# ishine/minimax-speech

Measured on AMD Instinct MI355X. Metric: 24 kHz audio-seconds generated per wall-second per node (CosyVoice2-0.5B-shaped LM + flow + DAC-VAE, end to end), higher is better.
Workload: dtype bf16

## Files before the change

include/mmx_hip.h:

```cpp
#ifndef MMX_HIP_H
#define MMX_HIP_H
#include <stdint.h>
#ifdef __cplusplus
extern "C" {
#endif

#ifndef __HIP__
typedef struct ihipStream_t* hipStream_t;
#endif

#define MMX_F32 0
#define MMX_BF16 1
#define MMX_X2 2
#define MMX_X3 3
#define MMX_X2W 0x12
#define MMX_X3W 0x13
#define MMX_H2 4
#define MMX_H2W 0x14

#define MMX_ACT_NONE 0
#define MMX_ACT_LRELU 1
#define MMX_ACT_GELU 2
#define MMX_ACT_SILU 3
#define MMX_ACT_MISH 4
#define MMX_ACT_TANH 5

int mmx_abi_version(void);

typedef struct MmxGemmParams {
    const void* A;
    const void* W;
    const float* bias;
    const float* residual;
    const float* rowmask;
    const float* alpha;
    float* out_f32;
    void* out_act;
    int64_t lda, ldw, ldr, ldo_f, ldo_a;
    int64_t a_bstride, w_bstride, r_bstride, rm_bstride, of_bstride, oa_bstride;
    int64_t row_off, row_lo, row_hi;
    int64_t out_off, out_len;
    int32_t M, N, batch;
    int32_t ntaps, cin, dil;
    int32_t bias_mod, alpha_mod, bias_per_row;
    int32_t act, act2;
    float slope;
    int32_t row_stride;
} MmxGemmParams;
int mmx_gemm_win(const MmxGemmParams* p, int dtype, hipStream_t stream);
#define MMX_TILE_128x128 1
#define MMX_TILE_128x64 2
#define MMX_TILE_64x64 3
#define MMX_TILE_32x64 4
int mmx_gemm_win_tile(const MmxGemmParams* p, int dtype, int tile, hipStream_t stream);

int mmx_rownorm(const float* x, int64_t ldx, int64_t x_bstride, int rows, int C, int batch,
                const float* gamma, const float* beta, float eps, int rms, int act,
                const float* rowmask, int64_t rm_bstride, const float* addvec, int64_t av_bstride,
                float* out_f32, int64_t ldo_f, int64_t of_bstride,
                void* out_act, int64_t ldo_a, int64_t oa_bstride, int dtype, hipStream_t stream);

int mmx_groupnorm(const float* x, int B, int T, int C, int groups, const float* gamma, const float* beta, float eps,
                  int act, const float* rowmask, void* out, int dtype, hipStream_t stream);

int mmx_act_rows(const float* x, int64_t rows, int C, int act, const float* rowmask, float* out_f32, void* out_act, int dtype,
                 hipStream_t stream);

int mmx_gather_rows(const int64_t* ids, int n, const float* table, int C, float scale, const float* rowmask,
                    float* out_f32, int64_t ldo_f, void* out_act, int64_t ldo_a, int dtype, hipStream_t stream);

int mmx_copy2d(const void* in, int in_dtype, int64_t ibs, int64_t irs, int64_t ics, int rep,
               void* out, int out_dtype, int64_t obs, int64_t ors, int64_t ocs,
               int rows, int cols, int batch, hipStream_t stream);

int mmx_est_pack(const float* x, int64_t x_bs, int x_mod, const float* mu, const float* spks, const float* cond, int B, int T, int C,
                 void* h, int64_t ldh, int dtype, hipStream_t stream);
int mmx_sinusoidal_emb(const float* t, int B, int dim, float scale, void* out, int dtype, hipStream_t stream);

int mmx_cfg_euler(float* x, const float* d_cond, const float* d_uncond, float cfg, float dt, int64_t n,
                  hipStream_t stream);

int mmx_attn_dense(const void* q, int64_t ldq, int64_t q_bs, const void* k, int64_t ldk, int64_t k_bs,
                   const void* v, int64_t ldv, int64_t v_bs, void* out, int64_t ldo, int64_t o_bs,
                   int B, int H, int D, int Tq, int Tk, float scale, const float* keymask, int64_t km_bs, int chunk,
                   const void* pos, int64_t ldp, const float* pos_u, const float* pos_v,
                   int head_stride, int q_begin, int dtype, hipStream_t stream);
int mmx_attn_flash_bf16(const void* q, int64_t ldq, int64_t q_bs, const void* k, int64_t ldk, int64_t k_bs,
                        const void* vt, int64_t ldvt, int64_t vt_bs, void* out, int64_t ldo, int64_t o_bs,
                        int B, int H, int T, float scale, const float* keymask, int64_t km_bs, int chunk, int q_begin,
                        const int32_t* klen, hipStream_t stream);
int mmx_attn_relpos_x(const float* q, int64_t ldq, int64_t q_bs, const float* k, int64_t ldk, int64_t k_bs, const float* v,
                      int64_t ldv, int64_t v_bs, const float* pos, int64_t ldp, const float* pos_u, const float* pos_v,
                      float* out, int64_t ldo, int64_t o_bs, int B, int H, int T, float scale, int chunk, const int32_t* klen,
                      hipStream_t stream);
int mmx_attn_flash_x(const float* q, int64_t ldq, int64_t q_bs, const float* k, int64_t ldk, int64_t k_bs,
                     const float* v, int64_t ldv, int64_t v_bs, float* out, int64_t ldo, int64_t o_bs,
                     int B, int H, int T, float scale, const float* keymask, int64_t km_bs, int chunk,
                     int q_begin, const int32_t* klen, hipStream_t stream);
int mmx_attn_flash_xs(const void* qk, int64_t ldqk, int64_t qk_bs, const void* vt, int64_t ldvt, int64_t vt_bs,
                      float* out, int64_t ldo, int64_t o_bs, int B, int H, int T, float scale, const float* keymask,
                      int64_t km_bs, int chunk, int q_begin, const int32_t* klen, int form, hipStream_t stream);
int mmx_attn_relpos_bf16(const void* q, int64_t ldq, int64_t q_bs, const void* k, int64_t ldk, int64_t k_bs,
                         const void* vt, int64_t ldvt, int64_t vt_bs, const void* pos, int64_t ldp,
                         const float* pos_u, const float* pos_v, void* out, int64_t ldo, int64_t o_bs,
                         int B, int H, int T, float scale, int chunk, const int32_t* klen, hipStream_t stream);

int mmx_attn_flash_fp8(const void* q, int64_t ldq, int64_t q_bs, const void* k, int64_t ldk, int64_t k_bs,
                       const void* vt, int64_t ldvt, int64_t vt_bs, void* out, int64_t ldo, int64_t o_bs,
                       int B, int H, int T, float scale, const float* keymask, int64_t km_bs, int chunk, int q_begin,
                       const int32_t* klen, hipStream_t stream);

int mmx_conv_cin1(const float* x, int64_t x_bs, int T, int C, int k, const float* w, const float* bias, float slope,
                  const float* alpha, float* out_f32, void* out_act, int batch, int dtype, hipStream_t stream);
int mmx_vae_sample(const float* ml, const float* noise, int64_t rows, int D, float* z, float* m, float* logs,
                   hipStream_t stream);
int mmx_mask_rows(void* x, int64_t rows, int C, const float* rowmask, int dtype, hipStream_t stream);
int mmx_prefetch4(const void* p0, int64_t n0, const void* p1, int64_t n1, const void* p2, int64_t n2, const void* p3, int64_t n3,
                  void* sink, int workgroups, hipStream_t stream);
int mmx_resample_linear(const float* x, int64_t rows, int T, int T2, float* out, hipStream_t stream);

int mmx_conv_cout1_tanh(const void* act, int64_t a_bs, int T, int C, int k, const float* w, const float* bias,
                        float slope, int use_tanh, float* out, int64_t o_bs, int batch, int dtype, hipStream_t stream);

#define MMX_X_PACKED 1
#define MMX_OUT_PACKED 2
int mmx_pack_skinny(const void* w, int64_t ldw, int N, int K, const float* kscale, int interleave_half,
                    void* wp, int dtype, hipStream_t stream);
int mmx_skinny_gemm(const void* x, int x_dtype, int64_t ldx, int B, int K, int N, const void* wp,
                    const float* bias, int rs, float eps, int epi, float* out_f32, int64_t ldo_f,
                    void* out_act, int64_t ldo_a, int dtype, int flags, const float* kgamma, hipStream_t stream);

int mmx_decode_prep(const float* x, int64_t ldx, int B, int K, const float* gamma, float* h, int64_t ldh, void* xs,
                    float* ssq, int dtype, hipStream_t stream);
int mmx_skinny2(const void* xs, int B, int K, int N, const void* wp, const float* bias, const float* ssq_in, float eps,
                int epi, float* out, int64_t ldo, void* xs_out, const float* gamma_next, float* ssq_out,
                int tiles_per_wg, int ksplit, float* part, int64_t part_floats, int32_t* tickets, int dtype,
                hipStream_t stream);

int mmx_rope_kv_store(const float* qkv, int64_t ldqkv, int64_t qkv_bs, int B, int rows, int Hq, int Hkv, int D,
                      const float* inv_freq, const int32_t* pos, void* q_out, int64_t ldq, int64_t q_bs,
                      void* kc, void* vc, const int32_t* block_table, int max_pages, int page,
                      int dtype, hipStream_t stream);
int mmx_paged_attn(const void* q, int64_t ldq, int64_t q_bs, int B, int rows, int Hq, int Hkv, int D, float scale,
                   const int32_t* pos, const void* kc, const void* vc, const int32_t* block_table, int max_pages,
                   int page, void* out, int64_t ldo, int64_t o_bs, int dtype, hipStream_t stream);
int mmx_decode_attn(const float* qkv, int64_t ldqkv, int B, int Hq, int Hkv, int D, const float* inv_freq,
                    const float* rope_tab, const int32_t* pos, void* kc, void* vc, const int32_t* block_table, int max_pages, int page,
                    float scale, void* out, int64_t ldo, int dtype, int out_packed, hipStream_t stream);
int mmx_swiglu(const float* gu, int64_t ldgu, int rows, int I, void* out, int64_t ldo, int dtype, hipStream_t stream);

int mmx_sample_step(const float* logits, int64_t ldl, int V, int B, int eos_id, int top_k, float top_p,
                    int win_size, float tau_r, uint64_t seed, int32_t* state, int32_t* out_tokens, int max_out,
                    int32_t* sampled, const int32_t* forced, const float* speech_emb, int E, float* next_x,
                    int64_t ldx, float* logp_out, hipStream_t stream);

typedef struct MmxEstNext {
    const void* wqkv;
    const float* n1g;
    const float* n1b;
    void* q_out;
    void* vt_out;
    int64_t q_bs, vt_bs;
    int32_t ldq, ldvt;
} MmxEstNext;
typedef struct MmxEstTailParams {
    const void* ao;
    float* x;
    const void* wo;
    const void* w1;
    const void* w2;
    const float* bo;
    const float* b1;
    const float* b2;
    const float* n3g;
    const float* n3b;
    const float* rowmask;
    void* act_out;
    int64_t ao_bs, x_bs, rm_bs, act_bs;
    int32_t ldao, act_ld, B, T;
    int32_t t_begin;
    float eps;
    MmxEstNext next;
} MmxEstTailParams;
typedef struct MmxEstResnetParams {
    const void* a_in;
    float* x;
    const void* w1;
    const void* w2;
    const void* wr;
    const float* b1;
    const float* g1;
    const float* be1;
    const float* b2;
    const float* g2;
    const float* be2;
    const float* br;
    const float* tv;
    const float* rowmask;
    int64_t a_bs, x_bs, tv_bs, rm_bs;
    int32_t lda, cin, B, T;
    int32_t t_begin;
    float eps;
    MmxEstNext next;
} MmxEstResnetParams;
int mmx_est_tail(const MmxEstTailParams* p, int dtype, int bm, int cfg, hipStream_t stream);
int mmx_est_resnet(const MmxEstResnetParams* p, int dtype, int bm, int cfg, hipStream_t stream);
typedef struct {
    const float* x;
    float* x_out;
    void* act_out;
    const void* w7;
    const void* w1;
    const float* b7;
    const float* b1;
    const float* a0;
    const float* a2;
    const float* alpha_next;
    const int32_t* lens;
    int64_t x_bs;
    int32_t B, T, C, dil;
    float slope;
} MmxDacRuParams;
int mmx_dac_ru(const MmxDacRuParams* p, int dtype, int bm, hipStream_t stream);

#ifdef __cplusplus
}
#endif
#endif
```

minimax-speech_amd/csrc/common.h:

```cpp
#pragma once
#include <hip/hip_runtime.h>
#include <stdint.h>

#ifndef MMX_LAB
#define MMX_LAB 0
#endif
constexpr bool LAB = MMX_LAB != 0;

#define MMX_OK 0
#define MMX_EARG (-1)
#define MMX_CHECK_ARG(c) do { if (!(c)) return MMX_EARG; } while (0)
#define MMX_LAUNCH_CHECK() do { hipError_t e_ = hipGetLastError(); if (e_ != hipSuccess) return -(int)e_ - 1000; } while (0)

#define MMX_ACT_DTYPE(d) ((d) >= 2 ? 0 : (d))

#define MMX_LDS_OPT_IN(fn, bytes)                                                                                   \
    do {                                                                                                            \
        if ((bytes) > 64 * 1024) {                                                                                  \
            static bool done_[64] = {};                                                                             \
            int dev_ = 0;                                                                                           \
            if (hipGetDevice(&dev_) != hipSuccess || dev_ < 0 || dev_ >= 64) return MMX_EARG;                       \
            if (!done_[dev_]) {                                                                                     \
                hipError_t e_ = hipFuncSetAttribute((const void*)(fn), hipFuncAttributeMaxDynamicSharedMemorySize, 160 * 1024); \
                if (e_ != hipSuccess) return -1000 - (int)e_;                                                       \
                done_[dev_] = true;                                                                                 \
            }                                                                                                       \
        }                                                                                                           \
    } while (0)

typedef unsigned short bf16_t;
typedef __attribute__((ext_vector_type(8))) short short8_t;
typedef __attribute__((ext_vector_type(4))) float float4_t;
typedef __attribute__((ext_vector_type(4))) short short4_t;

__device__ __forceinline__ float bf2f(bf16_t v) { return __uint_as_float(((unsigned)v) << 16); }
__device__ __forceinline__ bf16_t f2bf(float f) { return __builtin_bit_cast(unsigned short, (__bf16)f); }
__device__ __forceinline__ unsigned pack_bf16x2(float lo, float hi) {
    typedef __attribute__((ext_vector_type(2))) __bf16 bf16x2_t;
    typedef __attribute__((ext_vector_type(2))) float f32x2_t;
    bf16x2_t v = __builtin_convertvector(f32x2_t{lo, hi}, bf16x2_t);
    return __builtin_bit_cast(unsigned, v);
}

template <typename T> struct Cvt;
template <> struct Cvt<float> {
    static __device__ __forceinline__ float to_f(float v) { return v; }
    static __device__ __forceinline__ float from_f(float v) { return v; }
};
template <> struct Cvt<bf16_t> {
    static __device__ __forceinline__ float to_f(bf16_t v) { return bf2f(v); }
    static __device__ __forceinline__ bf16_t from_f(float v) { return f2bf(v); }
};

template <int CTRL>
__device__ __forceinline__ float dpp_f32(float v) {
    return __builtin_bit_cast(float, __builtin_amdgcn_update_dpp(0, __builtin_bit_cast(int, v), CTRL, 0xf, 0xf, false));
}
__device__ __forceinline__ float group8_sum(float v) {
    v += dpp_f32<0xB1>(v);
    v += dpp_f32<0x4E>(v);
    v += dpp_f32<0x141>(v);
    return v;
}
__device__ __forceinline__ float group16_sum(float v) {
    v = group8_sum(v);
    v += dpp_f32<0x140>(v);
    return v;
}

__device__ __forceinline__ float wave_sum(float v) {
#pragma unroll
    for (int o = 32; o > 0; o >>= 1) v += __shfl_xor(v, o, 64);
    return v;
}
__device__ __forceinline__ float wave_max(float v) {
#pragma unroll
    for (int o = 32; o > 0; o >>= 1) v = fmaxf(v, __shfl_xor(v, o, 64));
    return v;
}

enum { ACT_NONE = 0, ACT_LRELU = 1, ACT_GELU = 2, ACT_SILU = 3, ACT_MISH = 4, ACT_TANH = 5 };

__device__ __forceinline__ float erf_fast(float x) {
    const float ax = fabsf(x);
    const float t = __builtin_amdgcn_rcpf(1.0f + 0.3275911f * ax);
    float p = 1.061405429f;
    p = p * t - 1.453152027f;
    p = p * t + 1.421413741f;
    p = p * t - 0.284496736f;
    p = p * t + 0.254829592f;
    const float r = 1.0f - p * t * __expf(-ax * ax);
    return copysignf(r, x);
}

typedef float f32x2_t __attribute__((ext_vector_type(2)));
__device__ __forceinline__ f32x2_t gelu_fast2(f32x2_t v) {
#pragma clang fp contract(off)
    const f32x2_t x = v * 0.70710678118654752f;
    const f32x2_t ax = __builtin_elementwise_abs(x);
    const f32x2_t d = __builtin_elementwise_fma(ax, (f32x2_t)(0.3275911f), (f32x2_t)(1.0f));
    f32x2_t t;
    t.x = __builtin_amdgcn_rcpf(d.x);
    t.y = __builtin_amdgcn_rcpf(d.y);
    f32x2_t p = (f32x2_t)(1.061405429f);
    p = __builtin_elementwise_fma(p, t, (f32x2_t)(-1.453152027f));
    p = __builtin_elementwise_fma(p, t, (f32x2_t)(1.421413741f));
    p = __builtin_elementwise_fma(p, t, (f32x2_t)(-0.284496736f));
    p = __builtin_elementwise_fma(p, t, (f32x2_t)(0.254829592f));
    const f32x2_t m = (ax * ax) * -1.4426950408889634f;
    f32x2_t e;
    e.x = __builtin_amdgcn_exp2f(m.x);
    e.y = __builtin_amdgcn_exp2f(m.y);
    const f32x2_t r = __builtin_elementwise_fma(-(p * t), e, (f32x2_t)(1.0f));
    f32x2_t er;
    er.x = __builtin_copysignf(r.x, x.x);
    er.y = __builtin_copysignf(r.y, x.y);
    return (v * 0.5f) * (er + 1.0f);
}

__device__ __forceinline__ float erf_poly(float x) {
    const float u = __builtin_fminf(__builtin_fmaxf(x, -3.0f), 3.0f);
    const float t = u * u;
    float p = 4.074212256e-08f;
    p = p * t - 1.944823225e-06f;
    p = p * t + 4.106053166e-05f;
    p = p * t - 5.110369530e-04f;
    p = p * t + 4.235427827e-03f;
    p = p * t - 2.510286123e-02f;
    p = p * t + 1.110793352e-01f;
    p = p * t - 3.753148615e-01f;
    p = p * t + 1.128268480e+00f;
    return u * p;
}

constexpr int ACT_GELU_POLY = 100;

template <int ACT, bool PRECISE>
__device__ __forceinline__ float act_c(float v, float slope) {
    if constexpr (ACT == ACT_LRELU) return v > 0.f ? v : v * slope;
    else if constexpr (ACT == ACT_GELU_POLY) return 0.5f * v * (1.f + erf_poly(v * 0.70710678118654752f));
    else if constexpr (ACT == ACT_GELU) return 0.5f * v * (1.f + (PRECISE ? erff(v * 0.70710678118654752f) : erf_fast(v * 0.70710678118654752f)));
    else if constexpr (ACT == ACT_SILU) return v / (1.f + (PRECISE ? expf(-v) : __expf(-v)));
    else if constexpr (ACT == ACT_MISH) {
        if (v > 20.f) return v;
        const float e = PRECISE ? expf(v) : __expf(v);
        const float n = e * (e + 2.f);
        return v * (n / (n + 2.f));
    } else if constexpr (ACT == ACT_TANH) return tanhf(v);
    else return v;
}

template <bool PRECISE>
__device__ __forceinline__ float act_apply(float v, int act, float slope) {
    switch (act) {
        case ACT_LRELU: return v > 0.f ? v : v * slope;
        case ACT_GELU: return 0.5f * v * (1.f + erff(v * 0.70710678118654752f));
        case ACT_SILU: return v / (1.f + (PRECISE ? expf(-v) : __expf(-v)));
        case ACT_MISH: {
            float sp = v > 20.f ? v : log1pf(PRECISE ? expf(v) : __expf(v));
            return v * tanhf(sp);
        }
        case ACT_TANH: return tanhf(v);
        default: return v;
    }
}

__device__ __forceinline__ float sin_cw(float x) {
    const float n = __builtin_rintf(x * 0.318309886183790672f);
    float r = __builtin_fmaf(-n, 3.14159274101257324f, x);
    r = __builtin_fmaf(-n, -8.74227765734758577e-8f, r);
    const float t = r * r;
    float p = -2.3846693509e-08f;
    p = p * t + 2.7522619348e-06f;
    p = p * t - 1.9840804453e-04f;
    p = p * t + 8.3333300427e-03f;
    p = p * t - 1.6666667163e-01f;
    const float s = __builtin_fmaf(r * t, p, r);
    return (static_cast<int>(n) & 1) ? -s : s;
}

template <bool PRECISE>
__device__ __forceinline__ float snake_apply(float x, float alpha) {
    float s = PRECISE ? sin_cw(alpha * x) : __sinf(alpha * x);
    return x + (1.0f / (alpha + 1e-9f)) * (s * s);
}
```

minimax-speech_amd/csrc/decode.hip:

```cpp
#include "common.h"
#include "../../include/mmx_hip.h"

namespace {

typedef __attribute__((ext_vector_type(4))) unsigned int u32x4_t;
typedef __attribute__((ext_vector_type(8))) _Float16 half8_t;
constexpr float H2_WSCALE = 256.f;

__device__ __forceinline__ void st_sc1(float* p, float v) { __hip_atomic_store(p, v, __ATOMIC_RELAXED, __HIP_MEMORY_SCOPE_AGENT); }
__device__ __forceinline__ float ld_sc1(const float* p) { return __hip_atomic_load(p, __ATOMIC_RELAXED, __HIP_MEMORY_SCOPE_AGENT); }

constexpr unsigned OOB = 0x80000000u;
constexpr int SSQ_SLOTS = 64;

__device__ __forceinline__ int plane_index(int row, int col, int nkb) {
    return (((((row >> 4) * nkb + (col >> 5)) << 6) + (((col & 31) >> 3) << 4) + (row & 15)) << 3) + (col & 7);
}
template <int NS, bool F16 = false>
__device__ __forceinline__ void store_split(bf16_t* planes, int ps, int idx, float v) {
#pragma unroll
    for (int s = 0; s < NS; ++s) {
        if constexpr (F16) {
            const _Float16 h = (_Float16)v;
            planes[s * ps + idx] = __builtin_bit_cast(unsigned short, h);
            v -= (float)h;
        } else {
            const bf16_t h = f2bf(v);
            planes[s * ps + idx] = h;
            v -= bf2f(h);
        }
    }
}
template <bool F16>
__device__ __forceinline__ float4_t mma16(u32x4_t a, u32x4_t b, float4_t c) {
    if constexpr (F16) return __builtin_amdgcn_mfma_f32_16x16x32_f16(__builtin_bit_cast(half8_t, a), __builtin_bit_cast(half8_t, b), c, 0, 0, 0);
    else return __builtin_amdgcn_mfma_f32_16x16x32_bf16(__builtin_bit_cast(short8_t, a), __builtin_bit_cast(short8_t, b), c, 0, 0, 0);
}

struct Skinny3Args {
    const bf16_t* xs;
    const bf16_t* wp;
    const float* bias;
    const float* ssq_in;
    float* out;
    bf16_t* xs_out;
    const float* gamma_next;
    float* ssq_out;
    float* part;
    int* tickets;
    long ldo;
    int B, K, N, ntiles, kb_per_wg;
    float eps;
    unsigned wplane;
    float wscale;
};

__device__ unsigned long long* g_skinny_stamps = nullptr;
#define STAMP(i) do { if constexpr (LAB) { if (stamps && lane == 0) stamps[((blockIdx.y * gridDim.x + blockIdx.x) * 8 + wave) * 8 + (i)] = __builtin_amdgcn_s_memtime(); } } while (0)

template <int MT, int TW, int KPW, int EPI, int NS, int NWP = 1, bool F16 = false>
__global__ __launch_bounds__(512) void skinny3_kernel(Skinny3Args a) {
    unsigned long long* stamps = nullptr;
    unsigned long long t_entry = 0;
    if constexpr (LAB) { t_entry = __builtin_amdgcn_s_memtime(); stamps = g_skinny_stamps; }
    constexpr int NB = EPI == 1 ? 2 : 1;
    constexpr int PER = TW * NB * MT * 4;
    extern __shared__ __attribute__((aligned(16))) char smem[];
    float* red = reinterpret_cast<float*>(smem);
    float* rstd = red + 8 * PER * 64;
    const int lane = threadIdx.x & 63;
    const int wave = __builtin_amdgcn_readfirstlane(threadIdx.x >> 6);
    const int g = lane >> 4, l16 = lane & 15;
    const int J = gridDim.y, j = blockIdx.y;
    const int nkb = a.K >> 5;
    const int wkb0 = j * a.kb_per_wg, wkb1 = min(nkb, wkb0 + a.kb_per_wg);
    const int wn = wkb1 - wkb0;
    const int kb0 = wkb0 + ((wn * wave) >> 3), kb1 = wkb0 + ((wn * (wave + 1)) >> 3);
    const int tile0 = blockIdx.x * TW;
    const int ntiles = a.ntiles;

    STAMP(0);
    if constexpr (LAB) { if (stamps && lane == 0) stamps[((blockIdx.y * gridDim.x + blockIdx.x) * 8 + wave) * 8 + 7] = t_entry; }
    const auto w_rsrc = __builtin_amdgcn_make_buffer_rsrc(const_cast<bf16_t*>(a.wp), 0, 0x7fffffff, 0x00020000);
    const auto x_rsrc = __builtin_amdgcn_make_buffer_rsrc(const_cast<bf16_t*>(a.xs), 0, 0x7fffffff, 0x00020000);
    const unsigned voff = lane * 16;
    u32x4_t wf[NWP][TW][NB][KPW];
#pragma unroll
    for (int p2 = 0; p2 < NWP; ++p2)
#pragma unroll
        for (int t = 0; t < TW; ++t)
#pragma unroll
            for (int n = 0; n < NB; ++n)
#pragma unroll
                for (int i = 0; i < KPW; ++i) {
                    const bool ok = tile0 + t < ntiles && kb0 + i < kb1;
                    const unsigned so = ok ? ((unsigned)(((tile0 + t) * NB + n) * nkb + kb0 + i) << 10) + p2 * a.wplane : OOB;
                    wf[p2][t][n][i] = __builtin_amdgcn_raw_buffer_load_b128(w_rsrc, voff, so, 2);
                }
    u32x4_t xf[NS][KPW][MT];
#pragma unroll
    for (int s = 0; s < NS; ++s)
#pragma unroll
        for (int i = 0; i < KPW; ++i)
#pragma unroll
            for (int m = 0; m < MT; ++m) {
                const unsigned so = kb0 + i < kb1 ? ((unsigned)((s * MT + m) * nkb + kb0 + i) << 10) : OOB;
                xf[s][i][m] = __builtin_amdgcn_raw_buffer_load_b128(x_rsrc, voff, so, 0);
            }
    if (a.ssq_in) {
        const int row = threadIdx.x >> 4, part = threadIdx.x & 15;
        const float4 q = *reinterpret_cast<const float4*>(a.ssq_in + row * SSQ_SLOTS + part * 4);
        float sq = group16_sum((q.x + q.y) + (q.z + q.w));
        if (part == 0) rstd[row] = rsqrtf(sq / (float)a.K + a.eps);
    }
    constexpr int UNITS = TW * MT * 4, UPW = (UNITS + 7) / 8;
    float pre_bias[UPW], pre_gn[UPW], pre_res[UPW];
#pragma unroll
    for (int k = 0; k < UPW; ++k) {
        const int u = wave + 8 * k, t = u / (MT * 4), m = (u / 4) % MT, r = u & 3;
        const int row = m * 16 + 4 * g + r, ncol = (tile0 + t) * 16 + l16;
        const bool ok = u < UNITS && tile0 + t < ntiles && row < a.B && ncol < a.N;
        pre_bias[k] = (EPI != 1 && a.bias && ok) ? a.bias[ncol] : 0.f;
        pre_gn[k] = (EPI == 2 && a.gamma_next && ok) ? a.gamma_next[ncol] : 1.f;
        pre_res[k] = (EPI == 2 && ok) ? a.out[(long)row * a.ldo + ncol] : 0.f;
    }
    STAMP(1);
    if constexpr (LAB) { if (stamps) { asm volatile("s_waitcnt vmcnt(0)" ::: "memory"); STAMP(2); } }
    float4_t acc[TW][NB][MT];
#pragma unroll
    for (int t = 0; t < TW; ++t)
#pragma unroll
        for (int n = 0; n < NB; ++n)
#pragma unroll
            for (int m = 0; m < MT; ++m) acc[t][n][m] = float4_t{0.f, 0.f, 0.f, 0.f};
#pragma unroll
    for (int i = 0; i < KPW; ++i)
#pragma unroll
        for (int t = 0; t < TW; ++t)
#pragma unroll
            for (int n = 0; n < NB; ++n)
#pragma unroll
                for (int p2 = 0; p2 < NWP; ++p2) {
#pragma unroll
                    for (int m = 0; m < MT; ++m)
#pragma unroll
                        for (int s = 0; s < NS; ++s) {
                            if (s + p2 >= NS) continue;
                            acc[t][n][m] = mma16<F16>(xf[s][i][m], wf[p2][t][n][i], acc[t][n][m]);
                        }
                }
    {
        float* mine = red + wave * PER * 64 + lane;
#pragma unroll
        for (int t = 0; t < TW; ++t)
#pragma unroll
            for (int n = 0; n < NB; ++n)
#pragma unroll
                for (int m = 0; m < MT; ++m)
#pragma unroll
                    for (int r = 0; r < 4; ++r) mine[(((t * NB + n) * MT + m) * 4 + r) * 64] = acc[t][n][m][r];
    }
    STAMP(3);
    __syncthreads();
    STAMP(4);
    float sum[UPW][NB];
#pragma unroll
    for (int k = 0; k < UPW; ++k) {
        const int u = wave + 8 * k, t = u / (MT * 4), m = (u / 4) % MT, r = u & 3;
#pragma unroll
        for (int n = 0; n < NB; ++n) {
            float v = 0.f;
            if (u < UNITS) {
#pragma unroll
                for (int w2 = 0; w2 < 8; ++w2) v += red[w2 * PER * 64 + (((t * NB + n) * MT + m) * 4 + r) * 64 + lane];
            }
            sum[k][n] = v;
        }
    }
    if constexpr (EPI == 2) {
        if (J > 1) {
            int* flag = reinterpret_cast<int*>(rstd + 32);
#pragma unroll
            for (int k = 0; k < UPW; ++k) {
                const int u = wave + 8 * k;
                if (u < UNITS) st_sc1(a.part + ((j * gridDim.x + blockIdx.x) * UNITS + u) * 64 + lane, sum[k][0]);
            }
            asm volatile("s_waitcnt vmcnt(0)" ::: "memory");
            __syncthreads();
            if (threadIdx.x == 0) {
                const int old = __hip_atomic_fetch_add(a.tickets + blockIdx.x, 1, __ATOMIC_RELAXED, __HIP_MEMORY_SCOPE_AGENT);
                if (old == J - 1) __hip_atomic_store(a.tickets + blockIdx.x, 0, __ATOMIC_RELAXED, __HIP_MEMORY_SCOPE_AGENT);
                *flag = old == J - 1;
            }
            __syncthreads();
            STAMP(5);
            if (!*flag) return;
            constexpr int JMAX = 8;
            float pv[UPW][JMAX];
#pragma unroll
            for (int k = 0; k < UPW; ++k)
#pragma unroll
                for (int j2 = 0; j2 < JMAX; ++j2) {
                    const int u = min(wave + 8 * k, UNITS - 1), jc = min(j2, J - 1);
                    const float v = ld_sc1(a.part + ((jc * gridDim.x + blockIdx.x) * UNITS + u) * 64 + lane);
                    pv[k][j2] = j2 < J ? v : 0.f;
                }
#pragma unroll
            for (int k = 0; k < UPW; ++k) {
                float v = 0.f;
#pragma unroll
                for (int j2 = 0; j2 < JMAX; ++j2) v += pv[k][j2];
                sum[k][0] = v;
            }
        }
    }
    const int nkb_out = a.N >> 5;
    const int ps_out = MT * nkb_out * 512;
#pragma unroll
    for (int k = 0; k < UPW; ++k) {
        const int u = wave + 8 * k, t = u / (MT * 4), m = (u / 4) % MT, r = u & 3;
        if (u >= UNITS) break;
        const int row = m * 16 + 4 * g + r, tile = tile0 + t, ncol = tile * 16 + l16;
        const float sc = (a.ssq_in ? rstd[row] : 1.f) * a.wscale;
        const bool ok = tile < ntiles && row < a.B && ncol < a.N;
        if constexpr (EPI == 1) {
            const float gte = sum[k][0] * sc, up = sum[k][1] * sc;
            if (ok) store_split<NS, F16>(a.xs_out, ps_out, plane_index(row, ncol, nkb_out), gte / (1.f + expf(-gte)) * up);
        } else {
            float vv = sum[k][0] * sc + pre_bias[k];
            if constexpr (EPI == 2) vv += pre_res[k];
            if (ok) a.out[(long)row * a.ldo + ncol] = vv;
            if constexpr (EPI == 2) {
                if (ok && a.xs_out) store_split<NS, F16>(a.xs_out, ps_out, plane_index(row, ncol, nkb_out), vv * pre_gn[k]);
                if (a.ssq_out) {
                    const float q = group16_sum(ok ? vv * vv : 0.f);
                    if (l16 == 0 && tile < ntiles) a.ssq_out[row * SSQ_SLOTS + tile] = q;
                }
            }
        }
    }
    STAMP(6);
}

template <int MT, int TW, int KPW, int EPI, int NS, int NWP = 1, bool F16 = false>
int launch(const Skinny3Args& a, int J, hipStream_t s) {
    constexpr int NB = EPI == 1 ? 2 : 1;
    const size_t lds = (size_t)8 * (TW * NB * MT * 4) * 64 * sizeof(float) + 32 * sizeof(float) + 16;
    MMX_LDS_OPT_IN((skinny3_kernel<MT, TW, KPW, EPI, NS, NWP, F16>), lds);
    dim3 grid((a.ntiles + TW - 1) / TW, J);
    hipLaunchKernelGGL((skinny3_kernel<MT, TW, KPW, EPI, NS, NWP, F16>), grid, dim3(512), lds, s, a);
    MMX_LAUNCH_CHECK();
    return MMX_OK;
}

template <int NS, bool F16 = false>
__global__ __launch_bounds__(256) void decode_prep_kernel(const float* __restrict__ x, long ldx, int B, int K, const float* __restrict__ gamma,
                                                          float* __restrict__ h, long ldh, bf16_t* __restrict__ xs, int mt,
                                                          float* __restrict__ ssq) {
    const int row = blockIdx.x, nkb = K >> 5;
    const int ps = mt * nkb * 512;
    for (int t0 = threadIdx.x; t0 < SSQ_SLOTS * 16; t0 += 256) {
        const int tile = t0 >> 4, col = t0;
        float v = 0.f;
        if (col < K) {
            v = x[(long)row * ldx + col];
            if (h) h[(long)row * ldh + col] = v;
            store_split<NS, F16>(xs, ps, plane_index(row, col, nkb), v * (gamma ? gamma[col] : 1.f));
        }
        const float q = group16_sum(v * v);
        if ((t0 & 15) == 0) ssq[row * SSQ_SLOTS + tile] = q;
    }
}

}

extern "C" int mmx_decode_prep(const float* x, int64_t ldx, int B, int K, const float* gamma, float* h, int64_t ldh, void* xs,
                               float* ssq, int dtype, hipStream_t stream) {
    MMX_CHECK_ARG(x && xs && ssq && B > 0 && B <= 32 && K > 0 && K % 32 == 0 && K <= SSQ_SLOTS * 16 && (dtype == MMX_X3 || dtype == MMX_BF16 || dtype == MMX_H2));
    if (dtype == MMX_H2) hipLaunchKernelGGL((decode_prep_kernel<2, true>), dim3(B), dim3(256), 0, stream, x, ldx, B, K, gamma, h, ldh, (bf16_t*)xs, (B + 15) / 16, ssq);
    else if (dtype == MMX_X3) hipLaunchKernelGGL(decode_prep_kernel<3>, dim3(B), dim3(256), 0, stream, x, ldx, B, K, gamma, h, ldh, (bf16_t*)xs, (B + 15) / 16, ssq);
    else hipLaunchKernelGGL(decode_prep_kernel<1>, dim3(B), dim3(256), 0, stream, x, ldx, B, K, gamma, h, ldh, (bf16_t*)xs, (B + 15) / 16, ssq);
    MMX_LAUNCH_CHECK();
    return MMX_OK;
}

extern "C" int mmx_skinny2(const void* xs, int B, int K, int N, const void* wp, const float* bias, const float* ssq_in, float eps,
                           int epi, float* out, int64_t ldo, void* xs_out, const float* gamma_next, float* ssq_out,
                           int tiles_per_wg, int ksplit, float* part, int64_t part_floats, int32_t* tickets, int dtype,
                           hipStream_t stream) {
    MMX_CHECK_ARG(xs && wp && B > 0 && B <= 32 && K > 0 && K % 32 == 0 && N > 0 &&
                  (dtype == MMX_X3 || dtype == MMX_X3W || dtype == MMX_BF16 || dtype == MMX_H2 || dtype == MMX_H2W));
    MMX_CHECK_ARG(dtype != MMX_X3W || tiles_per_wg == 1);
    MMX_CHECK_ARG(((uintptr_t)xs % 16) == 0 && ((uintptr_t)wp % 16) == 0 && (!ssq_in || ((uintptr_t)ssq_in % 16) == 0));
    MMX_CHECK_ARG(ksplit >= 1 && ksplit <= 8 && (ksplit == 1 || (epi == 2 && part && tickets)));
    MMX_CHECK_ARG(epi == 1 ? (xs_out != nullptr && N % 32 == 0) : out != nullptr);
    MMX_CHECK_ARG(epi != 2 || !xs_out || N % 32 == 0);
    MMX_CHECK_ARG(epi != 2 || !ssq_out || (N + 15) / 16 <= SSQ_SLOTS);
    const int nkb = K / 32, ntiles = (N + 15) / 16, mt = (B + 15) / 16;
    const int per_wave = ((nkb + ksplit - 1) / ksplit + 7) / 8;
    MMX_CHECK_ARG(ksplit == 1 || part_floats >= (int64_t)ksplit * ((ntiles + tiles_per_wg - 1) / tiles_per_wg) * tiles_per_wg * mt * 4 * 64);
    const double plane_bytes = (double)ntiles * (epi == 1 ? 2 : 1) * nkb * 1024.0;
    MMX_CHECK_ARG(plane_bytes * (dtype == MMX_X3W ? 3 : (dtype == MMX_H2W ? 2 : 1)) < 2147483000.0);
    const bool f16 = dtype == MMX_H2 || dtype == MMX_H2W;
    Skinny3Args a{(const bf16_t*)xs, (const bf16_t*)wp, bias, ssq_in, out, (bf16_t*)xs_out, gamma_next, ssq_out, part, tickets,
                  ldo, B, K, N, ntiles, (nkb + ksplit - 1) / ksplit, eps, (unsigned)plane_bytes, f16 ? 1.0f / H2_WSCALE : 1.0f};
#define GO(MT, TW, KPW, EPI) do { if (dtype == MMX_X3) return launch<MT, TW, KPW, EPI, 3>(a, ksplit, stream); \
                                  if (dtype == MMX_H2) return launch<MT, TW, KPW, EPI, 2, 1, true>(a, ksplit, stream); \
                                  if (dtype == MMX_H2W) return launch<MT, TW, KPW, EPI, 2, 2, true>(a, ksplit, stream); \
                                  if (dtype == MMX_X3W) { if constexpr (TW == 1) return launch<MT, 1, KPW, EPI, 3, 3>(a, ksplit, stream); else return MMX_EARG; } \
                                  return launch<MT, TW, KPW, EPI, 1>(a, ksplit, stream); } while (0)
#define BY_MT(TW, KPW, EPI) do { if (mt == 1) GO(1, TW, KPW, EPI); else GO(2, TW, KPW, EPI); } while (0)
    if (per_wave <= 4) {
        if (epi == 0) { if (tiles_per_wg == 1) BY_MT(1, 4, 0); if (tiles_per_wg == 2) BY_MT(2, 4, 0); }
        if (epi == 1) { if (tiles_per_wg == 1) BY_MT(1, 4, 1); if (tiles_per_wg == 2) BY_MT(2, 4, 1); }
        if (epi == 2) { if (tiles_per_wg == 1) BY_MT(1, 4, 2); if (tiles_per_wg == 2) BY_MT(2, 4, 2); }
    }
#undef BY_MT
#undef GO
    return MMX_EARG;
}

#if MMX_LAB
extern "C" int mmx_lab_skinny_stamps(void* buf) {
    unsigned long long* p = reinterpret_cast<unsigned long long*>(buf);
    const hipError_t e = hipMemcpyToSymbol(HIP_SYMBOL(g_skinny_stamps), &p, sizeof(p));
    return e == hipSuccess ? MMX_OK : -(int)e - 1000;
}
#endif
```

minimax-speech_amd/csrc/llm.hip:

```cpp
#include "common.h"
#include "../../include/mmx_hip.h"

template <typename T>
__global__ void pack_skinny_kernel(const T* __restrict__ w, long ldw, int N, int K, const float* __restrict__ kscale,
                                   int half, T* __restrict__ wp) {
    constexpr int E = sizeof(T) == 2 ? 8 : 4;
    constexpr int KB = E * 4;
    const long total = (long)((N + 15) / 16) * (K / KB) * 64 * E;
    for (long idx = (long)blockIdx.x * blockDim.x + threadIdx.x; idx < total; idx += (long)gridDim.x * blockDim.x) {
        int j = idx % E;
        long t = idx / E;
        int lane = t % 64;
        t /= 64;
        int kb = t % (K / KB);
        int tile = t / (K / KB);
        int col = lane & 15, g = lane >> 4;
        int row;
        if (half > 0) row = (tile & 1) * half + (tile >> 1) * 16 + col;
        else row = tile * 16 + col;
        int kk = kb * KB + g * E + j;
        float v = 0.f;
        if (row < N && (half == 0 || ((tile >> 1) * 16 + col) < half)) {
            v = Cvt<T>::to_f(w[(long)row * ldw + kk]);
            if (kscale) v *= kscale[kk];
        }
        wp[idx] = Cvt<T>::from_f(v);
    }
}
extern "C" int mmx_pack_skinny(const void* w, int64_t ldw, int N, int K, const float* kscale, int interleave_half,
                               void* wp, int dtype, hipStream_t stream) {
    MMX_CHECK_ARG(w && wp && N > 0 && K > 0 && K % 32 == 0);
    MMX_CHECK_ARG(interleave_half == 0 || (N == 2 * interleave_half && interleave_half % 16 == 0));
    if (dtype == MMX_X2 || dtype == MMX_X3) { MMX_CHECK_ARG(!kscale); dtype = MMX_BF16; }
    if (dtype == MMX_BF16) hipLaunchKernelGGL(pack_skinny_kernel<bf16_t>, dim3(2048), dim3(256), 0, stream, (const bf16_t*)w, ldw, N, K, kscale, interleave_half, (bf16_t*)wp);
    else if (dtype == MMX_F32) hipLaunchKernelGGL(pack_skinny_kernel<float>, dim3(2048), dim3(256), 0, stream, (const float*)w, ldw, N, K, kscale, interleave_half, (float*)wp);
    else return MMX_EARG;
    MMX_LAUNCH_CHECK();
    return MMX_OK;
}

template <typename T>
__device__ __forceinline__ long act_packed_index(int row, int col, int K) {
    constexpr int E = sizeof(T) == 2 ? 8 : 4, KB = 4 * E;
    const int kb = col / KB, g = (col % KB) / E, j = col % E;
    return ((((long)(row >> 4) * (K / KB) + kb) * 64) + g * 16 + (row & 15)) * E + j;
}

template <typename T, typename TX, int MT, int EPI, int KS, bool XPK, bool OPK, int NS = 1>
__global__ __launch_bounds__(512) void skinny_gemm_kernel(const TX* __restrict__ x, long ldx, int B, int K, int N,
                                   const T* __restrict__ wp, const float* __restrict__ bias, int rs, float eps,
                                   float* __restrict__ outf, long ldo_f, T* __restrict__ outa, long ldo_a,
                                   int ksplit, int ntiles, const float* __restrict__ kgamma) {
    constexpr bool BF = sizeof(T) == 2;
    static_assert(NS == 1 || (BF && sizeof(TX) == 4 && !XPK && !OPK), "split build: bf16 weights, fp32 row-major activations");
    constexpr int E = BF ? 8 : 4;
    constexpr int KB = E * 4;
    constexpr int NB = EPI == 1 ? 2 : 1;
    constexpr int XV = sizeof(TX) == 4 ? E / 4 : 1;
    typedef __attribute__((ext_vector_type(4))) unsigned int u32x4_t;
    extern __shared__ __attribute__((aligned(16))) char smem[];
    float* red = reinterpret_cast<float*>(smem);
    const int lane = threadIdx.x & 63, wave = threadIdx.x >> 6;
    const int nwaves = blockDim.x >> 6;
    const int g = lane >> 4, l16 = lane & 15;
    const int tpb = nwaves / ksplit;
    const int tile = blockIdx.x * tpb + wave / ksplit;
    const int ksl = wave % ksplit;
    const int nkb = K / KB;
    const int kb_per = (nkb + ksplit - 1) / ksplit;
    const int kb0 = ksl * kb_per, kb1 = min(nkb, kb0 + kb_per);
    const bool active = tile < ntiles;

    float4_t acc[NB][MT];
#pragma unroll
    for (int n = 0; n < NB; ++n)
#pragma unroll
        for (int m = 0; m < MT; ++m) acc[n][m] = float4_t{0.f, 0.f, 0.f, 0.f};
    float ssq[MT];
#pragma unroll
    for (int m = 0; m < MT; ++m) ssq[m] = 0.f;
    constexpr bool SSQ_MFMA = BF && sizeof(TX) == 2 && EPI != 2;
    float4_t accd[MT];
#pragma unroll
    for (int m = 0; m < MT; ++m) accd[m] = float4_t{0.f, 0.f, 0.f, 0.f};
    float pre_bias = 0.f, pre_res[MT][4];
    if (active && ksl == 0) {
        const int n = tile * 16 + l16;
        if (EPI != 1 && bias && n < N) pre_bias = bias[n];
        if constexpr (EPI == 2) {
#pragma unroll
            for (int m = 0; m < MT; ++m)
#pragma unroll
                for (int r = 0; r < 4; ++r) {
                    const int row = m * 16 + 4 * g + r;
                    pre_res[m][r] = (row < B && n < N) ? outf[(long)row * ldo_f + n] : 0.f;
                }
        }
    }

    if (active) {
        const T* wbase = wp + ((long)tile * NB * nkb) * 64 * E + (long)lane * E;
        for (int kc = kb0; kc < kb1; kc += KS) {
            u32x4_t wf[KS][NB];
#pragma unroll
            for (int i = 0; i < KS; ++i)
#pragma unroll
                for (int n = 0; n < NB; ++n)
                    if (kc + i < kb1)
                        wf[i][n] = __builtin_nontemporal_load(reinterpret_cast<const u32x4_t*>(wbase + ((long)n * nkb + kc + i) * 64 * E));
            u32x4_t xr[KS][MT][XV];
#pragma unroll
            for (int i = 0; i < KS; ++i)
#pragma unroll
                for (int m = 0; m < MT; ++m)
#pragma unroll
                    for (int v = 0; v < XV; ++v) {
                        if constexpr (XPK)
                            xr[i][m][v] = (kc + i < kb1)
                                              ? *reinterpret_cast<const u32x4_t*>(x + (((long)m * nkb + kc + i) * 64 + lane) * E)
                                              : u32x4_t{0, 0, 0, 0};
                        else
                            xr[i][m][v] = (kc + i < kb1 && m * 16 + l16 < B)
                                              ? *reinterpret_cast<const u32x4_t*>(reinterpret_cast<const char*>(x + (long)(m * 16 + l16) * ldx + (kc + i) * KB + g * E) + v * 16)
                                              : u32x4_t{0, 0, 0, 0};
                    }
#pragma unroll
            for (int i = 0; i < KS; ++i) {
                if (kc + i >= kb1) continue;
#pragma unroll
                for (int m = 0; m < MT; ++m) {
                    float xv[E];
                    u32x4_t raw[XV];
#pragma unroll
                    for (int v = 0; v < XV; ++v) raw[v] = xr[i][m][v];
                    if constexpr (sizeof(TX) == 4) {
#pragma unroll
                        for (int e = 0; e < E; ++e) xv[e] = __uint_as_float(raw[e / 4][e % 4]);
                    } else {
#pragma unroll
                        for (int e = 0; e < E; ++e) xv[e] = __uint_as_float((raw[0][e / 2] >> ((e & 1) * 16)) << 16);
                    }
                    if constexpr (SSQ_MFMA) {
                        if (rs) {
                            const short8_t xf = *reinterpret_cast<const short8_t*>(&raw[0]);
                            accd[m] = __builtin_amdgcn_mfma_f32_16x16x32_bf16(xf, xf, accd[m], 0, 0, 0);
                        }
                    } else if (rs) {
#pragma unroll
                        for (int e = 0; e < E; ++e) ssq[m] += xv[e] * xv[e];
                    }
                    if constexpr (NS > 1 || (BF && sizeof(TX) == 4)) {
                        if (kgamma) {
                            const float4 g0 = *reinterpret_cast<const float4*>(kgamma + (kc + i) * KB + g * E);
                            const float4 g1 = *reinterpret_cast<const float4*>(kgamma + (kc + i) * KB + g * E + 4);
                            xv[0] *= g0.x; xv[1] *= g0.y; xv[2] *= g0.z; xv[3] *= g0.w;
                            xv[4] *= g1.x; xv[5] *= g1.y; xv[6] *= g1.z; xv[7] *= g1.w;
                        }
#pragma unroll
                        for (int s2 = 0; s2 < NS; ++s2) {
                            short8_t af;
#pragma unroll
                            for (int e = 0; e < 8; ++e) {
                                const bf16_t hb = f2bf(xv[e]);
                                af[e] = (short)hb;
                                xv[e] -= bf2f(hb);
                            }
#pragma unroll
                            for (int n = 0; n < NB; ++n) {
                                short8_t bfr = *reinterpret_cast<const short8_t*>(&wf[i][n]);
                                acc[n][m] = __builtin_amdgcn_mfma_f32_16x16x32_bf16(af, bfr, acc[n][m], 0, 0, 0);
                            }
                        }
                    } else if constexpr (BF) {
                        short8_t af;
                        if constexpr (sizeof(TX) == 2) {
                            af = *reinterpret_cast<const short8_t*>(&raw[0]);
                        } else {
#pragma unroll
                            for (int e = 0; e < 8; ++e) af[e] = (short)f2bf(xv[e]);
                        }
#pragma unroll
                        for (int n = 0; n < NB; ++n) {
                            short8_t bfr = *reinterpret_cast<const short8_t*>(&wf[i][n]);
                            acc[n][m] = __builtin_amdgcn_mfma_f32_16x16x32_bf16(af, bfr, acc[n][m], 0, 0, 0);
                        }
                    } else {
#pragma unroll
                        for (int n = 0; n < NB; ++n) {
                            float4_t bfr = *reinterpret_cast<const float4_t*>(&wf[i][n]);
#pragma unroll
                            for (int s2 = 0; s2 < 4; ++s2)
                                acc[n][m] = __builtin_amdgcn_mfma_f32_16x16x4f32(xv[s2], bfr[s2], acc[n][m], 0, 0, 0);
                        }
                    }
                }
            }
        }
    }
    if constexpr (SSQ_MFMA) {
        if (rs) {
#pragma unroll
            for (int m = 0; m < MT; ++m) {
                const int r = l16 & 3;
                const float d = r == 0 ? accd[m][0] : (r == 1 ? accd[m][1] : (r == 2 ? accd[m][2] : accd[m][3]));
                ssq[m] = (l16 >> 2) == g ? d : 0.f;
            }
        }
    }
    if (rs) {
#pragma unroll
        for (int m = 0; m < MT; ++m) {
            ssq[m] += __shfl_xor(ssq[m], 16, 64);
            ssq[m] += __shfl_xor(ssq[m], 32, 64);
        }
    }
    constexpr int PER = NB * MT * 4 + MT;
    if (ksplit > 1) {
        float* mine = red + ((long)wave * PER) * 64 + lane;
#pragma unroll
        for (int n = 0; n < NB; ++n)
#pragma unroll
            for (int m = 0; m < MT; ++m)
#pragma unroll
                for (int r = 0; r < 4; ++r) mine[((n * MT + m) * 4 + r) * 64] = acc[n][m][r];
#pragma unroll
        for (int m = 0; m < MT; ++m) mine[(NB * MT * 4 + m) * 64] = ssq[m];
        __syncthreads();
        if (ksl != 0) return;
        for (int w2 = 1; w2 < ksplit; ++w2) {
            const float* o = red + ((long)(wave + w2) * PER) * 64 + lane;
#pragma unroll
            for (int n = 0; n < NB; ++n)
#pragma unroll
                for (int m = 0; m < MT; ++m)
#pragma unroll
                    for (int r = 0; r < 4; ++r) acc[n][m][r] += o[((n * MT + m) * 4 + r) * 64];
#pragma unroll
            for (int m = 0; m < MT; ++m) ssq[m] += o[(NB * MT * 4 + m) * 64];
        }
    }
    if (!active) return;
#pragma unroll
    for (int m = 0; m < MT; ++m) {
#pragma unroll
        for (int r = 0; r < 4; ++r) {
            const int row = m * 16 + 4 * g + r;
            float sc = 1.f;
            if (rs) {
                float sq = __shfl(ssq[m], 4 * g + r, 64);
                sc = rsqrtf(sq / (float)K + eps);
            }
            if (row >= B) continue;
            if constexpr (EPI == 1) {
                const int n = tile * 16 + l16;
                if (n < N) {
                    float gte = acc[0][m][r] * sc, up = acc[1][m][r] * sc;
                    float sl = gte / (1.f + expf(-gte));
                    if constexpr (NS > 1) outf[(long)row * ldo_f + n] = sl * up;
                    else outa[OPK ? act_packed_index<T>(row, n, N) : (long)row * ldo_a + n] = Cvt<T>::from_f(sl * up);
                }
            } else {
                const int n = tile * 16 + l16;
                if (n < N) {
                    float v = acc[0][m][r] * sc + pre_bias;
                    if constexpr (EPI == 2) v += pre_res[m][r];
                    if (outf) outf[(long)row * ldo_f + n] = v;
                    if constexpr (NS == 1)
                        if (outa) outa[OPK ? act_packed_index<T>(row, n, N) : (long)row * ldo_a + n] = Cvt<T>::from_f(v);
                }
            }
        }
    }
}

template <typename T, typename TX, int EPI, bool XPK, bool OPK, int NS = 1>
static int skinny_launch_mt(const void* x, int64_t ldx, int B, int K, int N, const void* wp, const float* bias, int rs,
                            float eps, float* outf, int64_t ldo_f, void* outa, int64_t ldo_a, hipStream_t s,
                            const float* kgamma = nullptr) {
    constexpr int KB = sizeof(T) == 2 ? 32 : 16;
    const int ntiles = (N + 15) / 16;
    const int nkb = K / KB;
    const int mt = (B + 15) / 16;
    const int KSr = mt == 1 ? 10 : (mt == 2 ? 7 : 4);
    int ksplit = 1;
    while (ksplit < 8 && (nkb + ksplit - 1) / ksplit > KSr) ksplit *= 2;
    int waves = ksplit >= 4 ? ksplit : 4;
    if (mt >= 2 && ksplit <= 4 && ntiles >= 256) waves = 8;
    int tpb = waves / ksplit;
    dim3 grid((ntiles + tpb - 1) / tpb), block(waves * 64);
    constexpr int NB = EPI == 1 ? 2 : 1;
    size_t lds = ksplit > 1 ? (size_t)waves * (NB * mt * 4 + mt) * 64 * 4 : 0;
#define SK(MT) hipLaunchKernelGGL((skinny_gemm_kernel<T, TX, MT, EPI, (MT == 1 ? 10 : (MT == 2 ? 7 : 4)), XPK, OPK, NS>), grid, block, lds, s, (const TX*)x, ldx, B, K, N, (const T*)wp, \
        bias, rs, eps, outf, ldo_f, (T*)outa, ldo_a, ksplit, ntiles, kgamma)
    switch (mt) {
        case 1: SK(1); break;
        case 2: SK(2); break;
        case 3: SK(3); break;
        case 4: SK(4); break;
        default: return MMX_EARG;
    }
#undef SK
    MMX_LAUNCH_CHECK();
    return MMX_OK;
}
template <typename T, typename TX, bool XPK, bool OPK>
static int skinny_launch_epi(int epi, const void* x, int64_t ldx, int B, int K, int N, const void* wp, const float* bias,
                             int rs, float eps, float* outf, int64_t ldo_f, void* outa, int64_t ldo_a, hipStream_t s) {
    if (epi == 0) return skinny_launch_mt<T, TX, 0, XPK, OPK>(x, ldx, B, K, N, wp, bias, rs, eps, outf, ldo_f, outa, ldo_a, s);
    if (epi == 1) return skinny_launch_mt<T, TX, 1, XPK, OPK>(x, ldx, B, K, N, wp, bias, rs, eps, outf, ldo_f, outa, ldo_a, s);
    if (epi == 2) return skinny_launch_mt<T, TX, 2, XPK, OPK>(x, ldx, B, K, N, wp, bias, rs, eps, outf, ldo_f, outa, ldo_a, s);
    return MMX_EARG;
}
template <typename T, typename TX>
static int skinny_launch_layout(int flags, int epi, const void* x, int64_t ldx, int B, int K, int N, const void* wp,
                                const float* bias, int rs, float eps, float* outf, int64_t ldo_f, void* outa, int64_t ldo_a,
                                hipStream_t s) {
    if constexpr (sizeof(T) == sizeof(TX)) {
        if (flags == (MMX_X_PACKED | MMX_OUT_PACKED))
            return skinny_launch_epi<T, TX, true, true>(epi, x, ldx, B, K, N, wp, bias, rs, eps, outf, ldo_f, outa, ldo_a, s);
        if (flags == MMX_X_PACKED)
            return skinny_launch_epi<T, TX, true, false>(epi, x, ldx, B, K, N, wp, bias, rs, eps, outf, ldo_f, outa, ldo_a, s);
    }
    if (flags == 0) return skinny_launch_epi<T, TX, false, false>(epi, x, ldx, B, K, N, wp, bias, rs, eps, outf, ldo_f, outa, ldo_a, s);
    return MMX_EARG;
}
template <int NS>
static int skinny_launch_split(int epi, const void* x, int64_t ldx, int B, int K, int N, const void* wp, const float* bias, int rs,
                               float eps, float* outf, int64_t ldo_f, hipStream_t s, const float* kgamma) {
    if (epi == 0) return skinny_launch_mt<bf16_t, float, 0, false, false, NS>(x, ldx, B, K, N, wp, bias, rs, eps, outf, ldo_f, nullptr, 0, s, kgamma);
    if (epi == 1) return skinny_launch_mt<bf16_t, float, 1, false, false, NS>(x, ldx, B, K, N, wp, bias, rs, eps, outf, ldo_f, nullptr, 0, s, kgamma);
    if (epi == 2) return skinny_launch_mt<bf16_t, float, 2, false, false, NS>(x, ldx, B, K, N, wp, bias, rs, eps, outf, ldo_f, nullptr, 0, s, kgamma);
    return MMX_EARG;
}
extern "C" int mmx_skinny_gemm(const void* x, int x_dtype, int64_t ldx, int B, int K, int N, const void* wp,
                               const float* bias, int rs, float eps, int epi, float* out_f32, int64_t ldo_f,
                               void* out_act, int64_t ldo_a, int dtype, int flags, const float* kgamma, hipStream_t stream) {
    MMX_CHECK_ARG(x && wp && B > 0 && B <= 64 && K > 0 && K % 32 == 0 && N > 0);
    if (dtype == MMX_X2 || dtype == MMX_X3) {
        MMX_CHECK_ARG(x_dtype == MMX_F32 && flags == 0 && out_f32 && !out_act && ldx % 8 == 0 && ((uintptr_t)x % 16) == 0 && ((uintptr_t)wp % 16) == 0);
        MMX_CHECK_ARG(!kgamma || ((uintptr_t)kgamma % 16) == 0);
        return dtype == MMX_X2 ? skinny_launch_split<2>(epi, x, ldx, B, K, N, wp, bias, rs, eps, out_f32, ldo_f, stream, kgamma)
                               : skinny_launch_split<3>(epi, x, ldx, B, K, N, wp, bias, rs, eps, out_f32, ldo_f, stream, kgamma);
    }
    if (kgamma) {
        MMX_CHECK_ARG(dtype == MMX_BF16 && x_dtype == MMX_F32 && flags == 0 && ((uintptr_t)kgamma % 16) == 0 && ldx % 8 == 0 && ((uintptr_t)x % 16) == 0);
        if (epi == 0) return skinny_launch_mt<bf16_t, float, 0, false, false, 1>(x, ldx, B, K, N, wp, bias, rs, eps, out_f32, ldo_f, out_act, ldo_a, stream, kgamma);
        if (epi == 1) return skinny_launch_mt<bf16_t, float, 1, false, false, 1>(x, ldx, B, K, N, wp, bias, rs, eps, out_f32, ldo_f, out_act, ldo_a, stream, kgamma);
        return MMX_EARG;
    }
    MMX_CHECK_ARG((flags == 0 || flags == MMX_X_PACKED || flags == (MMX_X_PACKED | MMX_OUT_PACKED)) && (flags == 0 || x_dtype == dtype) &&
                  (!(flags & MMX_OUT_PACKED) || N % 32 == 0));
    MMX_CHECK_ARG(ldx % 8 == 0 && ((uintptr_t)x % 16) == 0 && ((uintptr_t)wp % 16) == 0);
    MMX_CHECK_ARG(epi == 1 ? out_act != nullptr : (out_f32 != nullptr || (epi == 0 && out_act != nullptr)));
    MMX_CHECK_ARG(epi != 2 || out_f32 != nullptr);
    if (dtype == MMX_BF16) {
        if (x_dtype == MMX_F32) return skinny_launch_layout<bf16_t, float>(flags, epi, x, ldx, B, K, N, wp, bias, rs, eps, out_f32, ldo_f, out_act, ldo_a, stream);
        if (x_dtype == MMX_BF16) return skinny_launch_layout<bf16_t, bf16_t>(flags, epi, x, ldx, B, K, N, wp, bias, rs, eps, out_f32, ldo_f, out_act, ldo_a, stream);
    } else if (dtype == MMX_F32 && x_dtype == MMX_F32) {
        return skinny_launch_layout<float, float>(flags, epi, x, ldx, B, K, N, wp, bias, rs, eps, out_f32, ldo_f, out_act, ldo_a, stream);
    }
    return MMX_EARG;
}

template <typename T>
__global__ void rope_kv_kernel(const float* __restrict__ qkv, long ldqkv, long qkv_bs, int Hq, int Hkv,
                               const float* __restrict__ inv_freq, const int32_t* __restrict__ pos,
                               T* __restrict__ q_out, long ldq, long q_bs, T* __restrict__ kc, T* __restrict__ vc,
                               const int32_t* __restrict__ block_table, int max_pages, int page) {
    constexpr int D = 64, HALF = 32;
    const int b = blockIdx.y, t = blockIdx.x;
    const int p = pos[b] + t;
    const float* src = qkv + (long)b * qkv_bs + (long)t * ldqkv;
    const int nh = Hq + 2 * Hkv;
    const int phys = block_table[(long)b * max_pages + p / page];
    const int slot = p % page;
    for (int i = threadIdx.x; i < nh * HALF; i += blockDim.x) {
        const int hh = i / HALF, d = i % HALF;
        const float x0 = src[hh * D + d], x1 = src[hh * D + d + HALF];
        float y0 = x0, y1 = x1;
        if (hh < Hq + Hkv) {
            const float ang = (float)p * inv_freq[d];
            const float c = cosf(ang), s = sinf(ang);
            y0 = x0 * c - x1 * s;
            y1 = x1 * c + x0 * s;
        }
        if (hh < Hq) {
            T* o = q_out + (long)b * q_bs + (long)t * ldq + hh * D;
            o[d] = Cvt<T>::from_f(y0);
            o[d + HALF] = Cvt<T>::from_f(y1);
        } else {
            const int hk = (hh - Hq) % Hkv;
            T* base = (hh < Hq + Hkv ? kc : vc) + (((long)phys * Hkv + hk) * page + slot) * D;
            base[d] = Cvt<T>::from_f(y0);
            base[d + HALF] = Cvt<T>::from_f(y1);
        }
    }
}
extern "C" int mmx_rope_kv_store(const float* qkv, int64_t ldqkv, int64_t qkv_bs, int B, int rows, int Hq, int Hkv, int D,
                                 const float* inv_freq, const int32_t* pos, void* q_out, int64_t ldq, int64_t q_bs,
                                 void* kc, void* vc, const int32_t* block_table, int max_pages, int page,
                                 int dtype, hipStream_t stream) {
    dtype = MMX_ACT_DTYPE(dtype);
    MMX_CHECK_ARG(qkv && inv_freq && pos && q_out && kc && vc && block_table && B > 0 && rows > 0 && D == 64 && page > 0);
    dim3 grid(rows, B);
    if (dtype == MMX_BF16) hipLaunchKernelGGL(rope_kv_kernel<bf16_t>, grid, dim3(256), 0, stream, qkv, ldqkv, qkv_bs, Hq, Hkv, inv_freq, pos, (bf16_t*)q_out, ldq, q_bs, (bf16_t*)kc, (bf16_t*)vc, block_table, max_pages, page);
    else if (dtype == MMX_F32) hipLaunchKernelGGL(rope_kv_kernel<float>, grid, dim3(256), 0, stream, qkv, ldqkv, qkv_bs, Hq, Hkv, inv_freq, pos, (float*)q_out, ldq, q_bs, (float*)kc, (float*)vc, block_table, max_pages, page);
    else return MMX_EARG;
    MMX_LAUNCH_CHECK();
    return MMX_OK;
}

template <typename T>
__global__ __launch_bounds__(256) void paged_attn_kernel(
    const T* __restrict__ q, long ldq, long q_bs, int Hq, int Hkv, float scale, const int32_t* __restrict__ pos,
    const T* __restrict__ kc, const T* __restrict__ vc, const int32_t* __restrict__ block_table, int max_pages,
    int page, T* __restrict__ out, long ldo, long o_bs) {
    constexpr int D = 64;
    extern __shared__ __attribute__((aligned(16))) char smem[];
    float* qs = reinterpret_cast<float*>(smem);
    float* red = qs + D;
    float* S = red + 8 + 4 * D;
    const int tid = threadIdx.x, lane = tid & 63, wave = tid >> 6;
    const int h = blockIdx.x, t = blockIdx.y, b = blockIdx.z;
    const int hk = h / (Hq / Hkv);
    const int ctx = pos[b] + t + 1;
    const int32_t* bt = block_table + (long)b * max_pages;
    if (tid < D) qs[tid] = Cvt<T>::to_f(q[(long)b * q_bs + (long)t * ldq + h * D + tid]);
    __syncthreads();
    float mx = -INFINITY;
    for (int j = tid; j < ctx; j += 256) {
        const T* kp = kc + (((long)bt[j / page] * Hkv + hk) * page + j % page) * D;
        float s = 0.f;
#pragma unroll
        for (int d = 0; d < D; ++d) s += qs[d] * Cvt<T>::to_f(kp[d]);
        s *= scale;
        S[j] = s;
        mx = fmaxf(mx, s);
    }
    mx = wave_max(mx);
    if (lane == 0) red[wave] = mx;
    __syncthreads();
    mx = fmaxf(fmaxf(red[0], red[1]), fmaxf(red[2], red[3]));
    float l = 0.f;
    for (int j = tid; j < ctx; j += 256) {
        float e = expf(S[j] - mx);
        S[j] = e;
        l += e;
    }
    l = wave_sum(l);
    if (lane == 0) red[4 + wave] = l;
    __syncthreads();
    l = red[4] + red[5] + red[6] + red[7];
    float acc = 0.f;
    for (int j = wave; j < ctx; j += 4) {
        const T* vp = vc + (((long)bt[j / page] * Hkv + hk) * page + j % page) * D;
        acc += S[j] * Cvt<T>::to_f(vp[lane]);
    }
    red[8 + wave * D + lane] = acc;
    __syncthreads();
    if (wave == 0) {
        float o = (red[8 + lane] + red[8 + D + lane]) + (red[8 + 2 * D + lane] + red[8 + 3 * D + lane]);
        out[(long)b * o_bs + (long)t * ldo + h * D + lane] = Cvt<T>::from_f(o / l);
    }
}
extern "C" int mmx_paged_attn(const void* q, int64_t ldq, int64_t q_bs, int B, int rows, int Hq, int Hkv, int D, float scale,
                              const int32_t* pos, const void* kc, const void* vc, const int32_t* block_table, int max_pages,
                              int page, void* out, int64_t ldo, int64_t o_bs, int dtype, hipStream_t stream) {
    dtype = MMX_ACT_DTYPE(dtype);
    MMX_CHECK_ARG(q && pos && kc && vc && block_table && out && B > 0 && rows > 0 && D == 64 && Hq % Hkv == 0 && page > 0);
    const size_t max_ctx = (size_t)max_pages * page;
    size_t lds = (64 + 8 + 4 * 64 + max_ctx) * 4;
    MMX_CHECK_ARG(lds <= 160 * 1024);
    dim3 grid(Hq, rows, B);
    if (dtype == MMX_BF16) hipLaunchKernelGGL(paged_attn_kernel<bf16_t>, grid, dim3(256), lds, stream, (const bf16_t*)q, ldq, q_bs, Hq, Hkv, scale, pos, (const bf16_t*)kc, (const bf16_t*)vc, block_table, max_pages, page, (bf16_t*)out, ldo, o_bs);
    else if (dtype == MMX_F32) hipLaunchKernelGGL(paged_attn_kernel<float>, grid, dim3(256), lds, stream, (const float*)q, ldq, q_bs, Hq, Hkv, scale, pos, (const float*)kc, (const float*)vc, block_table, max_pages, page, (float*)out, ldo, o_bs);
    else return MMX_EARG;
    MMX_LAUNCH_CHECK();
    return MMX_OK;
}

template <typename T>
__device__ __forceinline__ void load8(const T* p, float o[8]) {
    if constexpr (sizeof(T) == 2) {
        uint4 r = *reinterpret_cast<const uint4*>(p);
        const unsigned w[4] = {r.x, r.y, r.z, r.w};
#pragma unroll
        for (int i = 0; i < 4; ++i) {
            o[2 * i] = __uint_as_float(w[i] << 16);
            o[2 * i + 1] = __uint_as_float(w[i] & 0xffff0000u);
        }
    } else {
        float4 a = *reinterpret_cast<const float4*>(p), b = *reinterpret_cast<const float4*>(p + 4);
        o[0] = a.x; o[1] = a.y; o[2] = a.z; o[3] = a.w; o[4] = b.x; o[5] = b.y; o[6] = b.z; o[7] = b.w;
    }
}
template <typename T>
struct Raw8 {
    uint4 a, b;
    __device__ __forceinline__ void load(const T* p) {
        a = *reinterpret_cast<const uint4*>(p);
        if constexpr (sizeof(T) == 4) b = *reinterpret_cast<const uint4*>(p + 4);
    }
    __device__ __forceinline__ void to_float(float o[8]) const {
        const unsigned w[4] = {a.x, a.y, a.z, a.w};
        if constexpr (sizeof(T) == 2) {
#pragma unroll
            for (int i = 0; i < 4; ++i) {
                o[2 * i] = __uint_as_float(w[i] << 16);
                o[2 * i + 1] = __uint_as_float(w[i] & 0xffff0000u);
            }
        } else {
            const unsigned w2[4] = {b.x, b.y, b.z, b.w};
#pragma unroll
            for (int i = 0; i < 4; ++i) { o[i] = __uint_as_float(w[i]); o[4 + i] = __uint_as_float(w2[i]); }
        }
    }
};

template <typename T, int OM, int HP>
__global__ __launch_bounds__(256) void decode_attn_kernel(
    const float* __restrict__ qkv, long ldqkv, int Hq, int Hkv, const float* __restrict__ inv_freq,
    const float* __restrict__ rope_tab, const int32_t* __restrict__ pos, T* __restrict__ kc, T* __restrict__ vc,
    const int32_t* __restrict__ block_table, int max_pages, int page, float scale, T* __restrict__ out, long ldo,
    int nseq) {
    constexpr int D = 64, HALF = 32, NG = 32;
    extern __shared__ __attribute__((aligned(16))) char smem[];
    float* qs = reinterpret_cast<float*>(smem);
    float* kn = qs + HP * D;
    float* vn = kn + D;
    float* gm = vn + D;
    float* gl = gm + HP * NG;
    float* part = gl + HP * NG;
    int* bts = reinterpret_cast<int*>(part + HP * NG * D);
    const int tid = threadIdx.x;
    const int group = Hq / Hkv, nsub = (group + HP - 1) / HP;
    const int xcd = blockIdx.x & 7, slot = blockIdx.x >> 3;
    const int kvg = (slot / nsub) * 8 + xcd;
    if (kvg >= Hkv * nseq) return;
    const int b = kvg / Hkv, hk = kvg % Hkv, sub = slot % nsub;
    const int h0 = hk * group + sub * HP, nh = min(HP, group - sub * HP);
    const int32_t* bt = block_table + (long)b * max_pages;
    for (int i = tid; i < max_pages; i += 256) bts[i] = bt[i];
    const int p = pos[b];
    const float* src = qkv + (long)b * ldqkv;
    const float sc2 = scale * 1.44269504088896341f;
    if (tid < (HP + 1) * HALF) {
        const int which = tid >> 5, d = tid & 31;
        const float* x = src + (which < HP ? (h0 + min(which, nh - 1)) * D : (Hq + hk) * D);
        float c, s;
        if (rope_tab) {
            c = rope_tab[(long)p * D + d];
            s = rope_tab[(long)p * D + HALF + d];
        } else {
            const float ang = (float)p * inv_freq[d];
            c = cosf(ang);
            s = sinf(ang);
        }
        const float y0 = x[d] * c - x[d + HALF] * s, y1 = x[d + HALF] * c + x[d] * s;
        if (which < HP) { qs[which * D + d] = y0 * sc2; qs[which * D + d + HALF] = y1 * sc2; }
        else { kn[d] = Cvt<T>::to_f(Cvt<T>::from_f(y0)); kn[d + HALF] = Cvt<T>::to_f(Cvt<T>::from_f(y1)); }
    } else if (tid < (HP + 1) * HALF + D) {
        const int d = tid - (HP + 1) * HALF;
        vn[d] = Cvt<T>::to_f(Cvt<T>::from_f(src[(Hq + Hkv + hk) * D + d]));
    }
    __syncthreads();
    if (sub == 0 && tid < D) {
        const long o = (((long)bts[p / page] * Hkv + hk) * page + p % page) * D + tid;
        kc[o] = Cvt<T>::from_f(kn[tid]);
        vc[o] = Cvt<T>::from_f(vn[tid]);
    }
    const int kg = tid >> 3, dc = tid & 7;
    float qv[HP][8];
#pragma unroll
    for (int hp = 0; hp < HP; ++hp)
#pragma unroll
        for (int e = 0; e < 8; ++e) qv[hp][e] = qs[hp * D + dc * 8 + e];
    float m[HP], l[HP], acc[HP][8];
#pragma unroll
    for (int hp = 0; hp < HP; ++hp) {
        m[hp] = -INFINITY;
        l[hp] = 0.f;
#pragma unroll
        for (int e = 0; e < 8; ++e) acc[hp][e] = 0.f;
    }
    auto consume = [&](const float kv[8], const float vv[8]) {
#pragma unroll
        for (int hp = 0; hp < HP; ++hp) {
            float sdot = 0.f;
#pragma unroll
            for (int e = 0; e < 8; ++e) sdot = __builtin_fmaf(qv[hp][e], kv[e], sdot);
            sdot = group8_sum(sdot);
            const float mn = fmaxf(m[hp], sdot);
            const float al = __builtin_amdgcn_exp2f(m[hp] - mn), pj = __builtin_amdgcn_exp2f(sdot - mn);
            l[hp] = __builtin_fmaf(l[hp], al, pj);
#pragma unroll
            for (int e = 0; e < 8; ++e) acc[hp][e] = __builtin_fmaf(acc[hp][e], al, pj * vv[e]);
            m[hp] = mn;
        }
    };
    constexpr int U = sizeof(T) == 2 ? 12 : 10;
    for (int j0 = kg; j0 < p; j0 += NG * U) {
        Raw8<T> rk[U], rv[U];
#pragma unroll
        for (int u = 0; u < U; ++u) {
            const int j = j0 + u * NG;
            if (j < p) {
                const long o = (((long)bts[j / page] * Hkv + hk) * page + j % page) * D + dc * 8;
                rk[u].load(kc + o);
                rv[u].load(vc + o);
            }
        }
#pragma unroll
        for (int u = 0; u < U; ++u) {
            if (j0 + u * NG < p) {
                float kv[8], vv[8];
                rk[u].to_float(kv);
                rv[u].to_float(vv);
                consume(kv, vv);
            }
        }
    }
    if (kg == p % NG) {
        float kv[8], vv[8];
#pragma unroll
        for (int e = 0; e < 8; ++e) { kv[e] = kn[dc * 8 + e]; vv[e] = vn[dc * 8 + e]; }
        consume(kv, vv);
    }
#pragma unroll
    for (int hp = 0; hp < HP; ++hp) {
        if (dc == 0) { gm[hp * NG + kg] = m[hp]; gl[hp * NG + kg] = l[hp]; }
#pragma unroll
        for (int e = 0; e < 8; ++e) part[(hp * NG + kg) * D + dc * 8 + e] = acc[hp][e];
    }
    __syncthreads();
    if (tid < nh * D) {
        const int hp = tid >> 6, d = tid & 63, h = h0 + hp;
        const float* gmh = gm + hp * NG;
        const float* glh = gl + hp * NG;
        const float* ph = part + hp * NG * D;
        float M = -INFINITY;
#pragma unroll
        for (int g2 = 0; g2 < NG; ++g2) M = fmaxf(M, gmh[g2]);
        float L = 0.f, o = 0.f;
#pragma unroll
        for (int g2 = 0; g2 < NG; ++g2) {
            const float w = __builtin_amdgcn_exp2f(gmh[g2] - M);
            L = __builtin_fmaf(glh[g2], w, L);
            o = __builtin_fmaf(ph[g2 * D + d], w, o);
        }
        if constexpr (OM == 2) {
            const int nkb = Hq * D / 32, col = h * D + d;
            const long ps = (long)((nseq + 15) / 16) * nkb * 512;
            const long idx = ((((long)(b >> 4) * nkb + (col >> 5)) * 64) + (((col & 31) >> 3) << 4) + (b & 15)) * 8 + (col & 7);
            bf16_t* pl = reinterpret_cast<bf16_t*>(out);
            const float v = o / L;
            const bf16_t hh = f2bf(v);
            const float r1 = v - bf2f(hh);
            const bf16_t mm = f2bf(r1);
            pl[idx] = hh;
            pl[ps + idx] = mm;
            pl[2 * ps + idx] = f2bf(r1 - bf2f(mm));
        } else if constexpr (OM == 3) {
            const int nkb = Hq * D / 32, col = h * D + d;
            const long ps = (long)((nseq + 15) / 16) * nkb * 512;
            const long idx = ((((long)(b >> 4) * nkb + (col >> 5)) * 64) + (((col & 31) >> 3) << 4) + (b & 15)) * 8 + (col & 7);
            unsigned short* pl = reinterpret_cast<unsigned short*>(out);
            const float v = o / L;
            const _Float16 hh = (_Float16)v;
            pl[idx] = __builtin_bit_cast(unsigned short, hh);
            pl[ps + idx] = __builtin_bit_cast(unsigned short, (_Float16)(v - (float)hh));
        } else {
            out[OM == 1 ? act_packed_index<T>(b, h * D + d, Hq * D) : (long)b * ldo + h * D + d] = Cvt<T>::from_f(o / L);
        }
    }
}

template <bool OPK, int G>
__global__ __launch_bounds__(256) void decode_attn_gqa_kernel(
    const float* __restrict__ qkv, long ldqkv, int Hq, int Hkv, const float* __restrict__ inv_freq,
    const float* __restrict__ rope_tab, const int32_t* __restrict__ pos, bf16_t* __restrict__ kc, bf16_t* __restrict__ vc,
    const int32_t* __restrict__ block_table, int max_pages, float scale, bf16_t* __restrict__ out, long ldo, int nseq) {
    constexpr int D = 64, HALF = 32, PAGE = 16, NS = 8;
    static_assert(G <= 8, "one 8-float row of P per key");
    extern __shared__ __attribute__((aligned(16))) char smem[];
    bf16_t* qh = reinterpret_cast<bf16_t*>(smem);
    bf16_t* ql = qh + 16 * D;
    bf16_t* kn = ql + 16 * D;
    bf16_t* vn = kn + D;
    float* Pw = reinterpret_cast<float*>(vn + D);
    float* Aw = Pw + 4 * NS * 16 * 8;
    float* gm = Aw + 32;
    float* gl = gm + 32;
    float* part = gl + 32;
    int* bts = reinterpret_cast<int*>(part + 32 * G * D);
    const int tid = threadIdx.x, wave = tid >> 6, lane = tid & 63, l16 = lane & 15, g = lane >> 4;
    const int b = blockIdx.x / Hkv, hk = blockIdx.x % Hkv;
    const int32_t* bt = block_table + (long)b * max_pages;
    const int p = pos[b];
    const int NT = p / PAGE + 1;
    for (int i = tid; i < NT; i += 256) bts[i] = bt[i];
    for (int i = tid; i < 2 * 16 * D / 2; i += 256) reinterpret_cast<unsigned*>(qh)[i] = 0u;
    __syncthreads();
    const float* src = qkv + (long)b * ldqkv;
    const float sc2 = scale * 1.44269504088896341f;
    {
        const int which = tid >> 5, d = tid & 31;
        if (which <= G) {
            const float* x = src + (which < G ? (hk * G + which) * D : (Hq + hk) * D);
            float c, s;
            if (rope_tab) {
                c = rope_tab[(long)p * D + d];
                s = rope_tab[(long)p * D + HALF + d];
            } else {
                const float ang = (float)p * inv_freq[d];
                c = cosf(ang);
                s = sinf(ang);
            }
            const float y0 = x[d] * c - x[d + HALF] * s, y1 = x[d + HALF] * c + x[d] * s;
            if (which < G) {
                const float a0 = y0 * sc2, a1 = y1 * sc2;
                const bf16_t h0 = f2bf(a0), h1 = f2bf(a1);
                qh[which * D + d] = h0;
                qh[which * D + d + HALF] = h1;
                ql[which * D + d] = f2bf(a0 - bf2f(h0));
                ql[which * D + d + HALF] = f2bf(a1 - bf2f(h1));
            } else {
                kn[d] = f2bf(y0);
                kn[d + HALF] = f2bf(y1);
            }
        }
        if (tid < D) vn[tid] = f2bf(src[(Hq + Hkv + hk) * D + tid]);
    }
    __syncthreads();
    if (tid < D) {
        const long o = (((long)bts[p / PAGE] * Hkv + hk) * PAGE + p % PAGE) * D + tid;
        kc[o] = kn[tid];
        vc[o] = vn[tid];
    }
    short8_t bqh[2], bql[2];
#pragma unroll
    for (int ks = 0; ks < 2; ++ks) {
        bqh[ks] = *reinterpret_cast<const short8_t*>(qh + l16 * D + ks * 32 + 8 * g);
        bql[ks] = *reinterpret_cast<const short8_t*>(ql + l16 * D + ks * 32 + 8 * g);
    }
    const int ksub = lane >> 3, dc = lane & 7;
    const int tp = p / PAGE, rp = p % PAGE;
    float* Pme = Pw + wave * NS * 16 * 8;
    float m_run = -INFINITY, l_part = 0.f;
    typedef __attribute__((ext_vector_type(2))) float float2_t;
    float2_t acc[G][4];
#pragma unroll
    for (int h = 0; h < G; ++h)
#pragma unroll
        for (int e = 0; e < 4; ++e) acc[h][e] = float2_t{0.f, 0.f};

    for (int r0 = 0; r0 < NT; r0 += 4 * NS) {
        if (r0 + wave >= NT) break;
        uint4 rk[NS][2], rv[NS][2];
#pragma unroll
        for (int i = 0; i < NS; ++i) {
            const int t = r0 + 4 * i + wave;
            if (t < NT) {
                const long base = ((long)bts[t] * Hkv + hk) * PAGE * D;
#pragma unroll
                for (int ks = 0; ks < 2; ++ks) rk[i][ks] = *reinterpret_cast<const uint4*>(kc + base + l16 * D + ks * 32 + 8 * g);
#pragma unroll
                for (int hf = 0; hf < 2; ++hf) rv[i][hf] = *reinterpret_cast<const uint4*>(vc + base + (ksub + 8 * hf) * D + dc * 8);
            }
        }
        float4_t sacc[NS];
        float bm = -INFINITY;
#pragma unroll
        for (int i = 0; i < NS; ++i) {
            const int t = r0 + 4 * i + wave;
            sacc[i] = float4_t{-INFINITY, -INFINITY, -INFINITY, -INFINITY};
            if (t < NT) {
                if (t == tp) {
                    if (l16 == rp) {
#pragma unroll
                        for (int ks = 0; ks < 2; ++ks) rk[i][ks] = *reinterpret_cast<const uint4*>(kn + ks * 32 + 8 * g);
                    }
#pragma unroll
                    for (int hf = 0; hf < 2; ++hf) {
                        if (ksub + 8 * hf == rp) rv[i][hf] = *reinterpret_cast<const uint4*>(vn + dc * 8);
                        if (ksub + 8 * hf > rp) rv[i][hf] = make_uint4(0u, 0u, 0u, 0u);
                    }
                }
                float4_t c = {0.f, 0.f, 0.f, 0.f};
#pragma unroll
                for (int ks = 0; ks < 2; ++ks) {
                    const short8_t ak = __builtin_bit_cast(short8_t, rk[i][ks]);
                    c = __builtin_amdgcn_mfma_f32_16x16x32_bf16(ak, bqh[ks], c, 0, 0, 0);
                    c = __builtin_amdgcn_mfma_f32_16x16x32_bf16(ak, bql[ks], c, 0, 0, 0);
                }
#pragma unroll
                for (int r = 0; r < 4; ++r) {
                    const float x = (t * PAGE + 4 * g + r <= p) ? c[r] : -INFINITY;
                    sacc[i][r] = x;
                    bm = fmaxf(bm, x);
                }
            }
        }
        bm = fmaxf(bm, __shfl_xor(bm, 16, 64));
        bm = fmaxf(bm, __shfl_xor(bm, 32, 64));
        const float m_new = fmaxf(m_run, bm);
        const float alpha = __builtin_amdgcn_exp2f(m_run - m_new);
        m_run = m_new;
        float rs = 0.f;
#pragma unroll
        for (int i = 0; i < NS; ++i) {
            if (r0 + 4 * i + wave < NT) {
#pragma unroll
                for (int r = 0; r < 4; ++r) {
                    const float pj = __builtin_amdgcn_exp2f(sacc[i][r] - m_new);
                    rs += pj;
                    if (l16 < 8) Pme[(i * 16 + 4 * g + r) * 8 + l16] = pj;
                }
            }
        }
        l_part = l_part * alpha + rs;
        if (l16 < 8 && g == 0) Aw[wave * 8 + l16] = alpha;
        __builtin_amdgcn_fence(__ATOMIC_RELEASE, "wavefront");
        __builtin_amdgcn_wave_barrier();
        {
            const float4 a0 = *reinterpret_cast<const float4*>(Aw + wave * 8), a1 = *reinterpret_cast<const float4*>(Aw + wave * 8 + 4);
            const float al[8] = {a0.x, a0.y, a0.z, a0.w, a1.x, a1.y, a1.z, a1.w};
#pragma unroll
            for (int h = 0; h < G; ++h)
#pragma unroll
                for (int e = 0; e < 4; ++e) acc[h][e] *= al[h];
        }
#pragma unroll
        for (int i = 0; i < NS; ++i) {
            if (r0 + 4 * i + wave < NT) {
#pragma unroll
                for (int hf = 0; hf < 2; ++hf) {
                    const float* pr = Pme + (i * 16 + ksub + 8 * hf) * 8;
                    const float4 p0 = *reinterpret_cast<const float4*>(pr), p1 = *reinterpret_cast<const float4*>(pr + 4);
                    const float pv[8] = {p0.x, p0.y, p0.z, p0.w, p1.x, p1.y, p1.z, p1.w};
                    const unsigned w[4] = {rv[i][hf].x, rv[i][hf].y, rv[i][hf].z, rv[i][hf].w};
                    float2_t vv[4];
#pragma unroll
                    for (int e = 0; e < 4; ++e) vv[e] = float2_t{__uint_as_float(w[e] << 16), __uint_as_float(w[e] & 0xffff0000u)};
#pragma unroll
                    for (int h = 0; h < G; ++h) {
                        const float2_t ph = {pv[h], pv[h]};
#pragma unroll
                        for (int e = 0; e < 4; ++e) acc[h][e] = __builtin_elementwise_fma(ph, vv[e], acc[h][e]);
                    }
                }
            }
        }
        __builtin_amdgcn_fence(__ATOMIC_RELEASE, "wavefront");
        __builtin_amdgcn_wave_barrier();
    }
    l_part += __shfl_xor(l_part, 16, 64);
    l_part += __shfl_xor(l_part, 32, 64);
    if (l16 < 8 && g == 0) { gm[wave * 8 + l16] = m_run; gl[wave * 8 + l16] = l_part; }
#pragma unroll
    for (int h = 0; h < G; ++h) {
        float* pp = part + ((long)(wave * 8 + ksub) * G + h) * D + dc * 8;
        *reinterpret_cast<float4*>(pp) = make_float4(acc[h][0].x, acc[h][0].y, acc[h][1].x, acc[h][1].y);
        *reinterpret_cast<float4*>(pp + 4) = make_float4(acc[h][2].x, acc[h][2].y, acc[h][3].x, acc[h][3].y);
    }
    __syncthreads();
    for (int idx = tid; idx < G * D; idx += 256) {
        const int h = idx / D, d = idx % D;
        float M = -INFINITY;
#pragma unroll
        for (int w = 0; w < 4; ++w) M = fmaxf(M, gm[w * 8 + h]);
        float L = 0.f, o = 0.f;
#pragma unroll
        for (int w = 0; w < 4; ++w) {
            const float wt = __builtin_amdgcn_exp2f(gm[w * 8 + h] - M);
            L += gl[w * 8 + h] * wt;
            float sacc2 = 0.f;
#pragma unroll
            for (int k2 = 0; k2 < 8; ++k2) sacc2 += part[((long)(w * 8 + k2) * G + h) * D + d];
            o += sacc2 * wt;
        }
        const int col = (hk * G + h) * D + d;
        out[OPK ? act_packed_index<bf16_t>(b, col, Hq * D) : (long)b * ldo + col] = f2bf(o / L);
    }
}
extern "C" int mmx_decode_attn(const float* qkv, int64_t ldqkv, int B, int Hq, int Hkv, int D, const float* inv_freq,
                               const float* rope_tab, const int32_t* pos, void* kc, void* vc, const int32_t* block_table, int max_pages,
                               int page, float scale, void* out, int64_t ldo, int dtype, int out_packed, hipStream_t stream) {
    dtype = MMX_ACT_DTYPE(dtype);
    MMX_CHECK_ARG(qkv && (inv_freq || rope_tab) && pos && kc && vc && block_table && out && B > 0 && D == 64 && Hq % Hkv == 0 && page > 0);
    MMX_CHECK_ARG(out_packed >= 0 && out_packed <= 31);
    const bool gqa_shared = !(out_packed & 2);
    const bool split_out = out_packed & 4;
    const bool split_h2 = out_packed & 8;
    const bool one_head = (out_packed & 16) || (long)B * Hq <= 256;
    MMX_CHECK_ARG(!(split_out || split_h2) || (dtype == MMX_F32 && !(out_packed & 1) && !(split_out && split_h2)));
    out_packed &= 1;
    const size_t max_ctx = (size_t)max_pages * page;
    (void)max_ctx;
    const int hp = one_head ? 1 : 2, nsub = (Hq / Hkv + hp - 1) / hp;
    size_t lds = ((size_t)hp * 64 + 2 * 64 + 2 * hp * 32 + (size_t)hp * 32 * 64 + (size_t)max_pages) * 4;
    MMX_CHECK_ARG(lds <= 64 * 1024);
    dim3 grid(8 * ((Hkv * B + 7) / 8) * nsub);
#define DA(T, OM) do { if (one_head) hipLaunchKernelGGL((decode_attn_kernel<T, OM, 1>), grid, dim3(256), lds, stream, qkv, ldqkv, Hq, Hkv, inv_freq, rope_tab, pos, (T*)kc, (T*)vc, block_table, max_pages, page, scale, (T*)out, ldo, B); \
                       else hipLaunchKernelGGL((decode_attn_kernel<T, OM, 2>), grid, dim3(256), lds, stream, qkv, ldqkv, Hq, Hkv, inv_freq, rope_tab, pos, (T*)kc, (T*)vc, block_table, max_pages, page, scale, (T*)out, ldo, B); } while (0)
    if (dtype == MMX_BF16 && page == 16 && Hq == 7 * Hkv && gqa_shared) {
        const size_t lds2 = (2 * 16 * 64 + 2 * 64) * 2 + (4 * 8 * 16 * 8 + 3 * 32 + 32 * 7 * 64 + (size_t)max_pages) * 4;
        MMX_CHECK_ARG(lds2 <= 160 * 1024);
        if (out_packed) MMX_LDS_OPT_IN((decode_attn_gqa_kernel<true, 7>), lds2);
        else MMX_LDS_OPT_IN((decode_attn_gqa_kernel<false, 7>), lds2);
#define DG(OPK) hipLaunchKernelGGL((decode_attn_gqa_kernel<OPK, 7>), dim3(Hkv * B), dim3(256), lds2, stream, qkv, ldqkv, Hq, Hkv, inv_freq, rope_tab, pos, (bf16_t*)kc, (bf16_t*)vc, block_table, max_pages, scale, (bf16_t*)out, ldo, B)
        if (out_packed) DG(true); else DG(false);
    } else if (dtype == MMX_BF16) { if (out_packed) DA(bf16_t, 1); else DA(bf16_t, 0); }
    else if (dtype == MMX_F32) { if (split_h2) DA(float, 3); else if (split_out) DA(float, 2); else if (out_packed) DA(float, 1); else DA(float, 0); }
    else return MMX_EARG;
    MMX_LAUNCH_CHECK();
    return MMX_OK;
}
```

minimax-speech_amd/mmx/_lib.py:

```python
import ctypes as C
import os

import torch

F32, BF16 = 0, 1
X2, X3 = 2, 3
X2W, X3W = 0x12, 0x13
H2, H2W = 4, 0x14
ACT = {"none": 0, "lrelu": 1, "gelu": 2, "silu": 3, "mish": 4, "tanh": 5}
TORCH_DT = {F32: torch.float32, BF16: torch.bfloat16, X2: torch.float32, X3: torch.float32, X2W: torch.float32, X3W: torch.float32}
WEIGHT_DT = {F32: torch.float32, BF16: torch.bfloat16, X2: torch.bfloat16, X3: torch.bfloat16, X2W: torch.bfloat16, X3W: torch.bfloat16}
ESIZE = {F32: 4, BF16: 2, X2: 4, X3: 4}
WPLANES = {X2W: 2, X3W: 3}
DTYPE_NAMES = {"f32": F32, "bf16": BF16, "x": X2, "x2": X2, "x3": X3}


def is_split(dtype):
    return dtype in (X2, X3, X2W, X3W)

_HERE = os.path.dirname(os.path.abspath(__file__))
LIB_PATH = os.environ.get("MMX_LIB") or os.path.join(os.path.dirname(_HERE), "lib", "libmmx_hip.so")

SYMBOLS = [
    "mmx_abi_version", "mmx_gemm_win", "mmx_gemm_win_tile", "mmx_rownorm", "mmx_groupnorm", "mmx_act_rows", "mmx_gather_rows", "mmx_copy2d", "mmx_est_pack",
    "mmx_sinusoidal_emb", "mmx_cfg_euler", "mmx_attn_dense", "mmx_attn_flash_bf16", "mmx_attn_flash_fp8", "mmx_attn_relpos_bf16", "mmx_attn_relpos_x", "mmx_attn_flash_x", "mmx_attn_flash_xs", "mmx_conv_cout1_tanh", "mmx_conv_cin1", "mmx_vae_sample", "mmx_resample_linear", "mmx_prefetch4", "mmx_mask_rows",
    "mmx_est_tail", "mmx_est_resnet", "mmx_dac_ru", "mmx_pack_skinny", "mmx_skinny_gemm", "mmx_skinny2", "mmx_decode_prep", "mmx_rope_kv_store", "mmx_paged_attn", "mmx_decode_attn", "mmx_swiglu", "mmx_sample_step",
]


class GemmParams(C.Structure):
    _fields_ = [
        ("A", C.c_void_p), ("W", C.c_void_p), ("bias", C.c_void_p), ("residual", C.c_void_p),
        ("rowmask", C.c_void_p), ("alpha", C.c_void_p), ("out_f32", C.c_void_p), ("out_act", C.c_void_p),
        ("lda", C.c_int64), ("ldw", C.c_int64), ("ldr", C.c_int64), ("ldo_f", C.c_int64), ("ldo_a", C.c_int64),
        ("a_bstride", C.c_int64), ("w_bstride", C.c_int64), ("r_bstride", C.c_int64), ("rm_bstride", C.c_int64),
        ("of_bstride", C.c_int64), ("oa_bstride", C.c_int64),
        ("row_off", C.c_int64), ("row_lo", C.c_int64), ("row_hi", C.c_int64),
        ("out_off", C.c_int64), ("out_len", C.c_int64),
        ("M", C.c_int32), ("N", C.c_int32), ("batch", C.c_int32),
        ("ntaps", C.c_int32), ("cin", C.c_int32), ("dil", C.c_int32),
        ("bias_mod", C.c_int32), ("alpha_mod", C.c_int32), ("bias_per_row", C.c_int32),
        ("act", C.c_int32), ("act2", C.c_int32), ("slope", C.c_float), ("row_stride", C.c_int32),
    ]


class EstNext(C.Structure):
    _fields_ = [("wqkv", C.c_void_p), ("n1g", C.c_void_p), ("n1b", C.c_void_p), ("q_out", C.c_void_p), ("vt_out", C.c_void_p),
                ("q_bs", C.c_int64), ("vt_bs", C.c_int64), ("ldq", C.c_int32), ("ldvt", C.c_int32)]


class EstTailParams(C.Structure):
    _fields_ = [(k, C.c_void_p) for k in ("ao", "x", "wo", "w1", "w2", "bo", "b1", "b2", "n3g", "n3b", "rowmask", "act_out")] + \
               [(k, C.c_int64) for k in ("ao_bs", "x_bs", "rm_bs", "act_bs")] + \
               [(k, C.c_int32) for k in ("ldao", "act_ld", "B", "T", "t_begin")] + [("eps", C.c_float), ("next", EstNext)]


class EstResnetParams(C.Structure):
    _fields_ = [(k, C.c_void_p) for k in ("a_in", "x", "w1", "w2", "wr", "b1", "g1", "be1", "b2", "g2", "be2", "br", "tv", "rowmask")] + \
               [(k, C.c_int64) for k in ("a_bs", "x_bs", "tv_bs", "rm_bs")] + \
               [(k, C.c_int32) for k in ("lda", "cin", "B", "T", "t_begin")] + [("eps", C.c_float), ("next", EstNext)]


class DacRuParams(C.Structure):
    _fields_ = [(k, C.c_void_p) for k in ("x", "x_out", "act_out", "w7", "w1", "b7", "b1", "a0", "a2", "alpha_next", "lens")] + \
               [("x_bs", C.c_int64)] + [(k, C.c_int32) for k in ("B", "T", "C", "dil")] + [("slope", C.c_float)]


def fill_struct(st, **kw):
    for k, v in kw.items():
        if v is not None and hasattr(v, "data_ptr"):
            assert v.is_cuda
            v = v.data_ptr()
        setattr(st, k, v)
    return st


ABI_VERSION = 10
_lib = None


class MmxError(RuntimeError):
    pass


def load():
    global _lib
    if _lib is None:
        if not os.path.exists(LIB_PATH):
            raise MmxError(f"{LIB_PATH} not found: build it with `make -C minimax-speech_amd/csrc` "
                           "(or __graft_entry__.build()); the hot path has no CPU fallback")
        lib = C.CDLL(LIB_PATH)
        for s in SYMBOLS:
            getattr(lib, s).restype = C.c_int
        if lib.mmx_abi_version() != ABI_VERSION:
            raise MmxError(f"{LIB_PATH} has ABI version {lib.mmx_abi_version()}, this package binds version {ABI_VERSION}: "
                           "rebuild it (`make -C minimax-speech_amd/csrc`)")
        _lib = lib
    return _lib


def _p(t):
    if t is None:
        return None
    if isinstance(t, int):
        return C.c_void_p(t)
    assert t.is_cuda, "libmmx_hip works on device memory only (no CPU fallback)"
    return C.c_void_p(t.data_ptr())


def stream():
    return C.c_void_p(torch.cuda.current_stream().cuda_stream)


def check(rc, what):
    if rc != 0:
        raise MmxError(f"{what} failed with code {rc}" + (" (argument/shape error)" if rc == -1 else ""))


def dt_of(t):
    return BF16 if t.dtype == torch.bfloat16 else F32


def i64(x):
    return C.c_int64(int(x))


def gemm_params(**kw):
    p = GemmParams()
    p.bias_mod = 1
    p.alpha_mod = 1
    p.ntaps = 1
    p.dil = 1
    p.batch = 1
    p.row_lo = 0
    p.out_len = 1 << 62
    p.slope = 0.1
    p.row_stride = 1
    for k, v in kw.items():
        if k in ("A", "W", "bias", "residual", "rowmask", "alpha", "out_f32", "out_act"):
            v = None if v is None else (v if isinstance(v, int) else v.data_ptr())
        setattr(p, k, v)
    return p


TILES = {"auto": 0, "128x128": 1, "128x64": 2, "64x64": 3, "32x64": 4}


def gemm_win(p, dtype, tile=0):
    if tile:
        check(load().mmx_gemm_win_tile(C.byref(p), C.c_int(dtype), C.c_int(tile), stream()), "mmx_gemm_win_tile")
    else:
        check(load().mmx_gemm_win(C.byref(p), C.c_int(dtype), stream()), "mmx_gemm_win")
```

minimax-speech_amd/mmx/llm.py:

```python
import math
from typing import Dict, List, Optional

import torch

from . import ops
from ._lib import BF16, F32, H2, TORCH_DT, WEIGHT_DT, X3, X3W, is_split
from .flow import Graphed

ST_POS, ST_STEP, ST_NOUT, ST_FIN, ST_MINLEN, ST_MAXLEN, ST_SEQ, ST_ERR = range(8)


class PageAllocator:

    def __init__(self, n_pages: int):
        self.free_pages = list(range(n_pages - 1, -1, -1))
        self.n_pages = n_pages

    @property
    def n_free(self) -> int:
        return len(self.free_pages)

    def alloc(self, n: int) -> List[int]:
        if n > len(self.free_pages):
            raise RuntimeError(f"KV cache exhausted: {n} pages wanted, {len(self.free_pages)} free of {self.n_pages}")
        out = self.free_pages[-n:][::-1]
        del self.free_pages[-n:]
        return out

    def free(self, pages: List[int]):
        self.free_pages.extend(reversed(pages))


class LlmEngine:
    gqa_min_batch = 1 << 30
    use_v2 = True
    lm_planes = "f16x2"
    prefetch = 0

    def __init__(self, sd: Dict[str, torch.Tensor], dtype=BF16, device="cuda", max_batch=1, max_ctx=2048, page=16,
                 heads=14, kv_heads=2, head_dim=64, rope_theta=1e6, eps=1e-6, speech_token_size=6561, use_graphs=True,
                 prefix="llm.model.model", share_from=None, kv_pages=None, wplanes=False, lm_planes=None):
        self.dtype, self.tdt, self.dev = dtype, TORCH_DT[dtype], torch.device(device)
        self.wplanes = (dtype == X3 and ops.resolve_wplanes(wplanes, (v for k, v in sd.items() if v.dim() >= 2 and ("proj" in k or k == "llm_decoder.weight")))) \
            if share_from is None else share_from.wplanes
        planes = (lm_planes or self.lm_planes) if share_from is None else ("f16x2" if share_from.h2 else "bf16x3")
        assert planes in ("f16x2", "bf16x3")
        self.h2 = dtype == X3 and planes == "f16x2" and self.use_v2
        self.ddt = H2 if self.h2 else dtype
        if self.wplanes and not self.h2:
            self.v2_cfg = dict(qkv=(1, 1), o=(1, 1), gu=(1, 1), down=(1, 8), head=(1, 1))
        self.split = is_split(dtype)
        self.Hq, self.Hkv, self.D, self.eps = heads, kv_heads, head_dim, eps
        self.page, self.use_graphs = page, use_graphs
        self.eos = speech_token_size
        self.V = speech_token_size + 3
        dt = dtype
        if share_from is not None:
            o = share_from
            for k in ("n_layers", "H", "I", "layers", "wdec", "bdec", "embed_tokens", "speech_emb", "llm_emb", "inv_freq",
                      "rope_tab", "kc", "vc", "max_pages", "max_out", "trash_page", "pf_layers", "norm_w", "pages", "unfolded"):
                setattr(self, k, getattr(o, k))
            self.B = max_batch
            self.block_table = torch.full((self.B, self.max_pages), self.trash_page, dtype=torch.int32, device=self.dev)
            self.slot_pages = [[] for _ in range(self.B)]
            self._alloc_state()
            return
        f = lambda k: sd[k].detach().to(self.dev, torch.float32).contiguous()
        c = (lambda t: t.float().contiguous()) if self.wplanes else (lambda t: t.to(WEIGHT_DT[dtype]).contiguous())
        if self.wplanes:
            dt = X3W
        self.unfolded = dtype != F32
        ks = (lambda g: None) if self.unfolded else (lambda g: g)
        self.n_layers = len({k.split(".")[4] for k in sd if k.startswith(prefix + ".layers.")})
        self.H = sd[prefix + ".norm.weight"].shape[0]
        self.I = sd[prefix + ".layers.0.mlp.gate_proj.weight"].shape[0]
        self.layers, self.pf_layers = [], []
        for l in range(self.n_layers):
            p = f"{prefix}.layers.{l}"
            a = p + ".self_attn"
            wqkv = torch.cat([f(a + ".q_proj.weight"), f(a + ".k_proj.weight"), f(a + ".v_proj.weight")], 0)
            bqkv = torch.cat([f(a + ".q_proj.bias"), f(a + ".k_proj.bias"), f(a + ".v_proj.bias")], 0).contiguous()
            wgu = torch.cat([f(p + ".mlp.gate_proj.weight"), f(p + ".mlp.up_proj.weight")], 0)
            if max_batch >= 4 or self.wplanes or self.h2:
                self.pf_layers.append(dict(
                    wqkv=ops.pack_linear(c(wqkv), dt), wo=ops.pack_linear(c(f(a + ".o_proj.weight")), dt),
                    wgu=ops.pack_linear(c(wgu), dt), wdown=ops.pack_linear(c(f(p + ".mlp.down_proj.weight")), dt),
                    g1=f(p + ".input_layernorm.weight"), g2=f(p + ".post_attention_layernorm.weight")))
            if self.h2:
                pk = lambda w, ih=0: ops.pack_skinny_h2(w, planes=(2 if self.wplanes else 1), interleave_half=ih)
                self.layers.append(dict(wqkv=pk(wqkv), bqkv=bqkv, wo=pk(f(a + ".o_proj.weight")), wgu=pk(wgu, self.I),
                                        wdown=pk(f(p + ".mlp.down_proj.weight")),
                                        g1=f(p + ".input_layernorm.weight"), g2=f(p + ".post_attention_layernorm.weight")))
                del wqkv, wgu
                continue
            self.layers.append(dict(
                wqkv=ops.pack_skinny(c(wqkv), dtype=dt, kscale=ks(f(p + ".input_layernorm.weight"))), bqkv=bqkv,
                wo=ops.pack_skinny(c(f(a + ".o_proj.weight")), dtype=dt),
                wgu=ops.pack_skinny(c(wgu), dtype=dt, kscale=ks(f(p + ".post_attention_layernorm.weight")), interleave_half=self.I),
                wdown=ops.pack_skinny(c(f(p + ".mlp.down_proj.weight")), dtype=dt),
                g1=f(p + ".input_layernorm.weight"), g2=f(p + ".post_attention_layernorm.weight")))
            del wqkv, wgu
        self.norm_w = f(prefix + ".norm.weight")
        self.embed_tokens = f(prefix + ".embed_tokens.weight")
        if "llm_decoder.weight" in sd:
            self.wdec = ops.pack_skinny_h2(f("llm_decoder.weight"), planes=(2 if self.wplanes else 1)) if self.h2 else \
                ops.pack_skinny(c(f("llm_decoder.weight")), dtype=dt, kscale=ks(self.norm_w))
            self.bdec = f("llm_decoder.bias")
            self.speech_emb = f("speech_embedding.weight")
            self.llm_emb = f("llm_embedding.weight")
        else:
            self.wdec = self.bdec = self.speech_emb = self.llm_emb = None
        self.inv_freq = (1.0 / (rope_theta ** (torch.arange(0, head_dim, 2, dtype=torch.int64).float() / head_dim))).to(self.dev)
        self.max_pages = (max_ctx + page - 1) // page
        max_ctx = self.max_pages * page
        ang = torch.arange(max_ctx, dtype=torch.float32)[:, None] * self.inv_freq.cpu()[None, :]
        self.rope_tab = torch.cat([ang.cos(), ang.sin()], dim=1).contiguous().to(self.dev)
        self.B = max_batch
        npages = self.B * self.max_pages if kv_pages is None else int(kv_pages)
        self.trash_page = npages
        self.kc = torch.zeros(self.n_layers, npages + 1, kv_heads, page, head_dim, dtype=self.tdt, device=self.dev)
        self.vc = torch.zeros_like(self.kc)
        self.pages = PageAllocator(npages)
        self.block_table = torch.full((self.B, self.max_pages), self.trash_page, dtype=torch.int32, device=self.dev)
        self.slot_pages = [[] for _ in range(self.B)]
        self.max_out = max_ctx
        self._alloc_state()

    def _alloc_state(self):
        B = self.B
        self.state = torch.zeros(8, B, dtype=torch.int32, device=self.dev)
        self.out_tokens = torch.zeros(B, self.max_out, dtype=torch.int32, device=self.dev)
        self.sampled = torch.full((B, self.max_out), -1, dtype=torch.int32, device=self.dev)
        self.forced, self._forced_buf = None, None
        self.x_in = torch.zeros(B, self.H, device=self.dev)
        self.h = torch.zeros(B, self.H, device=self.dev)
        self.packed = B >= 4 and not self.unfolded
        self.h_act = torch.zeros(ops.packed_rows(B), self.H, dtype=self.tdt, device=self.dev)
        self.logits = torch.zeros(B, self.V, device=self.dev)
        self.logp = torch.zeros(B, self.V, device=self.dev)
        self.want_logp = False
        self.seed = 0
        self.top_p, self.top_k, self.win_size, self.tau_r = 0.8, 25, 10, 0.1
        self._decode = None
        self.reserve_ahead = 1 << 30

    def _layers(self, h, ha, B, rows, pos, block_table, packed=False):
        dt, H, I = self.dtype, self.H, self.I
        n = B * rows
        assert n <= 64 and not (packed and rows != 1)
        if self.split:
            return self._layers_split(h, B, rows, pos, block_table)
        nr = ops.packed_rows(n) if packed else n
        qkv = torch.empty(n, (self.Hq + 2 * self.Hkv) * self.D, device=self.dev)
        q = torch.empty(n, self.Hq * self.D, dtype=self.tdt, device=self.dev)
        att = torch.empty(nr, self.Hq * self.D, dtype=self.tdt, device=self.dev)
        act = torch.empty(nr, I, dtype=self.tdt, device=self.dev)
        pk = packed
        kg = (lambda g: g) if self.unfolded else (lambda g: None)
        for l, w in enumerate(self.layers):
            first = (packed and l == 0) or self.unfolded
            ops.skinny_gemm(h if first else ha, w["wqkv"], B=n, K=H, N=qkv.shape[1], dtype=dt, bias=w["bqkv"], rs=True,
                            eps=self.eps, epi=0, out_f32=qkv, x_packed=pk and not first, kgamma=kg(w["g1"]))
            if rows == 1:
                ops.decode_attn(qkv, self.inv_freq, pos, self.kc[l], self.vc[l], block_table, att, B=B, Hq=self.Hq,
                                Hkv=self.Hkv, page=self.page, dtype=dt, rope_tab=self.rope_tab, out_packed=pk,
                                per_head=B < self.gqa_min_batch)
            else:
                ops.rope_kv_store(qkv, self.inv_freq, pos, q, self.kc[l], self.vc[l], block_table, B=B, rows=rows,
                                  Hq=self.Hq, Hkv=self.Hkv, page=self.page, dtype=dt)
                ops.paged_attn(q, pos, self.kc[l], self.vc[l], block_table, att, B=B, rows=rows, Hq=self.Hq,
                               Hkv=self.Hkv, page=self.page, dtype=dt)
            ops.skinny_gemm(att, w["wo"], B=n, K=self.Hq * self.D, N=H, dtype=dt, epi=2, out_f32=h, out_act=ha,
                            x_packed=pk, out_packed=pk)
            ops.skinny_gemm(h if self.unfolded else ha, w["wgu"], B=n, K=H, N=I, dtype=dt, rs=True, eps=self.eps, epi=1, out_act=act,
                            x_packed=pk, out_packed=pk, kgamma=kg(w["g2"]))
            ops.skinny_gemm(act, w["wdown"], B=n, K=I, N=H, dtype=dt, epi=2, out_f32=h, out_act=ha,
                            x_packed=pk, out_packed=pk)

    v2_cfg = dict(qkv=(1, 1), o=(1, 1), gu=(2, 1), down=(2, 8), head=(2, 1))

    def _planes(self):
        if not hasattr(self, "_v2"):
            H, I, R = self.H, self.I, ops.packed_rows(self.B)
            NQ = (self.Hq + 2 * self.Hkv) * self.D
            bf = lambda K: torch.zeros((2 if self.h2 else 3) if self.split else 1, R * K, dtype=torch.bfloat16, device=self.dev)
            J = self.v2_cfg["down"][1]
            self._v2 = dict(qkv=torch.empty(self.B, NQ, device=self.dev), xs_a=bf(H), xs_b=bf(H), xs_att=bf(self.Hq * self.D), xs_act=bf(I),
                            ssq_a=torch.zeros(32, ops.SSQ_SLOTS, device=self.dev), ssq_b=torch.zeros(32, ops.SSQ_SLOTS, device=self.dev),
                            part=torch.empty(J * ((H + 15) // 16) * (R // 4) * 64, device=self.dev),
                            tickets=torch.zeros((H + 15) // 16, dtype=torch.int32, device=self.dev))
        return self._v2

    def _layers_split_decode(self, x_in, h, B, pos, block_table):
        dt, H, I, c, S = self.ddt, self.H, self.I, self.v2_cfg, self._planes()
        NQ = (self.Hq + 2 * self.Hkv) * self.D
        qkv = S["qkv"][:B]
        ops.decode_prep(x_in, S["xs_a"], S["ssq_a"], B=B, K=H, gamma=self.layers[0]["g1"], h=h, dtype=dt)
        pf = int(self.prefetch)
        if pf:
            if not hasattr(self, "_pf_side"):
                self._pf_side = torch.cuda.Stream(device=self.dev)
                self._pf_sink = torch.zeros(4, dtype=torch.int32, device=self.dev)
            cur, side = torch.cuda.current_stream(), self._pf_side
        for l, w in enumerate(self.layers):
            if pf:
                nxt = self.layers[l + 1] if l + 1 < len(self.layers) else None
                ev = torch.cuda.Event()
                ev.record(cur)
                side.wait_event(ev)
                with torch.cuda.stream(side):
                    ops.prefetch4([nxt["wqkv"], nxt["wo"], nxt["wgu"], nxt["wdown"]] if nxt is not None else [self.wdec], self._pf_sink, pf)
            g_next = self.layers[l + 1]["g1"] if l + 1 < len(self.layers) else self.norm_w
            ops.skinny2(S["xs_a"], w["wqkv"], B=B, K=H, N=NQ, dtype=dt, bias=w["bqkv"], ssq_in=S["ssq_a"], eps=self.eps, epi=0, out=qkv,
                        tiles_per_wg=c["qkv"][0])
            ops.decode_attn(qkv, self.inv_freq, pos, self.kc[l], self.vc[l], block_table, S["xs_att"], B=B, Hq=self.Hq,
                            Hkv=self.Hkv, page=self.page, dtype=self.dtype, rope_tab=self.rope_tab, per_head=(self.split or B < self.gqa_min_batch),
                            out_split=("f16" if self.h2 else self.split), out_packed=not self.split)
            ops.skinny2(S["xs_att"], w["wo"], B=B, K=self.Hq * self.D, N=H, dtype=dt, epi=2, out=h, xs_out=S["xs_b"],
                        gamma_next=w["g2"], ssq_out=S["ssq_b"], tiles_per_wg=c["o"][0])
            ops.skinny2(S["xs_b"], w["wgu"], B=B, K=H, N=I, dtype=dt, ssq_in=S["ssq_b"], eps=self.eps, epi=1, xs_out=S["xs_act"],
                        tiles_per_wg=c["gu"][0])
            ops.skinny2(S["xs_act"], w["wdown"], B=B, K=I, N=H, dtype=dt, epi=2, out=h, xs_out=S["xs_a"], gamma_next=g_next,
                        ssq_out=S["ssq_a"], tiles_per_wg=c["down"][0], ksplit=c["down"][1], part=S["part"], tickets=S["tickets"])
        if pf:
            ev = torch.cuda.Event()
            ev.record(side)
            cur.wait_event(ev)

    def _layers_split(self, h, B, rows, pos, block_table):
        dt, H, I = self.dtype, self.H, self.I
        n = B * rows
        qkv = torch.empty(n, (self.Hq + 2 * self.Hkv) * self.D, device=self.dev)
        q = torch.empty(n, self.Hq * self.D, device=self.dev)
        att = torch.empty(n, self.Hq * self.D, device=self.dev)
        act = torch.empty(n, I, device=self.dev)
        for l, w in enumerate(self.layers):
            ops.skinny_gemm(h, w["wqkv"], B=n, K=H, N=qkv.shape[1], dtype=dt, bias=w["bqkv"], rs=True, eps=self.eps, epi=0,
                            out_f32=qkv, kgamma=w["g1"])
            if rows == 1:
                ops.decode_attn(qkv, self.inv_freq, pos, self.kc[l], self.vc[l], block_table, att, B=B, Hq=self.Hq,
                                Hkv=self.Hkv, page=self.page, dtype=dt, rope_tab=self.rope_tab, per_head=True)
            else:
                ops.rope_kv_store(qkv, self.inv_freq, pos, q, self.kc[l], self.vc[l], block_table, B=B, rows=rows,
                                  Hq=self.Hq, Hkv=self.Hkv, page=self.page, dtype=dt)
                ops.paged_attn(q, pos, self.kc[l], self.vc[l], block_table, att, B=B, rows=rows, Hq=self.Hq,
                               Hkv=self.Hkv, page=self.page, dtype=dt)
            ops.skinny_gemm(att, w["wo"], B=n, K=self.Hq * self.D, N=H, dtype=dt, epi=2, out_f32=h)
            ops.skinny_gemm(h, w["wgu"], B=n, K=H, N=I, dtype=dt, rs=True, eps=self.eps, epi=1, out_f32=act, kgamma=w["g2"])
            ops.skinny_gemm(act, w["wdown"], B=n, K=I, N=H, dtype=dt, epi=2, out_f32=h)

    def _tail(self, B, packed=False, planes_ready=False):
        if self.unfolded and B <= 32 and self.use_v2:
            S = self._planes()
            if not planes_ready:
                ops.decode_prep(self.h, S["xs_a"], S["ssq_a"], B=B, K=self.H, gamma=self.norm_w, dtype=self.ddt)
            ops.skinny2(S["xs_a"], self.wdec, B=B, K=self.H, N=self.V, dtype=self.ddt, bias=self.bdec, ssq_in=S["ssq_a"],
                        eps=self.eps, epi=0, out=self.logits, tiles_per_wg=self.v2_cfg["head"][0])
        elif self.unfolded:
            ops.skinny_gemm(self.h, self.wdec, B=B, K=self.H, N=self.V, dtype=self.dtype, bias=self.bdec, rs=True,
                            eps=self.eps, epi=0, out_f32=self.logits, kgamma=self.norm_w)
        else:
            ops.skinny_gemm(self.h_act, self.wdec, B=B, K=self.H, N=self.V, dtype=self.dtype, bias=self.bdec, rs=True,
                            eps=self.eps, epi=0, out_f32=self.logits, x_packed=packed)
        ops.sample_step(self.logits, self.state, self.out_tokens, self.speech_emb, self.x_in, V=self.V, B=B,
                        eos_id=self.eos, seed=self.seed, top_k=self.top_k, top_p=self.top_p, win_size=self.win_size,
                        tau_r=self.tau_r, sampled=self.sampled, forced=self.forced,
                        logp_out=(self.logp if self.want_logp else None))

    def _decode_step(self):
        B = self.B
        if self.unfolded and B <= 32 and self.use_v2:
            self._layers_split_decode(self.x_in, self.h, B, self.state[ST_POS], self.block_table)
            return self._tail(B, planes_ready=True)
        self.h.copy_(self.x_in)
        if not self.packed:
            self.h_act[:B].copy_(self.x_in)
        self._layers(self.h, self.h_act, B, 1, self.state[ST_POS], self.block_table, packed=self.packed)
        self._tail(B, packed=self.packed)

    def build_lm_input(self, text, prompt_text, prompt_speech_token, speaker_embed=None):
        tok = torch.cat([prompt_text.reshape(-1), text.reshape(-1)]).to(self.dev, torch.int64)
        s = 0 if speaker_embed is None else 1
        L = 2 + s + tok.numel() + prompt_speech_token.numel()
        x = torch.empty(L, self.H, device=self.dev)
        x[0].copy_(self.llm_emb[0])
        if s:
            x[1].copy_(speaker_embed.reshape(-1))
        ops.gather_rows(tok, self.embed_tokens, out_f32=x[1 + s:1 + s + tok.numel()], dtype=F32)
        x[1 + s + tok.numel()].copy_(self.llm_emb[1])
        if prompt_speech_token.numel():
            ops.gather_rows(prompt_speech_token.reshape(-1).to(self.dev, torch.int64), self.speech_emb,
                            out_f32=x[2 + s + tok.numel():], dtype=F32)
        return x

    def speaker_conditioning(self, sd_linear_w, sd_linear_b, emb192):
        import math
        d = emb192.shape[1]
        g = torch.full((d,), 1.0 / math.sqrt(d), device=self.dev)
        en = torch.empty(1, d, dtype=self.tdt, device=self.dev)
        ops.rownorm(emb192.to(self.dev, torch.float32).contiguous(), g, None, 1e-30, rows=1, C_=d, rms=True, out_act=en, dtype=self.dtype)
        out = torch.empty(1, self.H, device=self.dev)
        ops.linear(en, sd_linear_w, d, dtype=self.dtype, bias=sd_linear_b, out_f32=out)
        return out

    def _set_pages(self, slot: int, rows: int):
        need = min((rows + self.page - 1) // self.page, self.max_pages)
        have = self.slot_pages[slot]
        if need > len(have):
            new = self.pages.alloc(need - len(have))
            self.block_table[slot, len(have):need] = torch.tensor(new, dtype=torch.int32)
            have.extend(new)

    def release(self, slot: int):
        if self.slot_pages[slot]:
            self.pages.free(self.slot_pages[slot])
            self.slot_pages[slot] = []
            self.block_table[slot].fill_(self.trash_page)

    def ensure_capacity(self, ahead: int, pos: Optional[List[int]] = None, active: Optional[List[int]] = None):
        pos = self.state[ST_POS].tolist() if pos is None else pos
        for s_ in (range(self.B) if active is None else active):
            if self.slot_pages[s_]:
                self._set_pages(s_, pos[s_] + 1 + ahead)

    @torch.no_grad()
    def admit(self, slot: int, x: torch.Tensor, min_len: int, max_len: int, seq_id: int, ahead: Optional[int] = None):
        L = x.shape[0]
        if L + max_len > self.max_pages * self.page:
            raise RuntimeError("sequence exceeds the KV cache")
        self.release(slot)
        self._set_pages(slot, L + (max_len if ahead is None else min(ahead, max_len)))
        x = x.to(self.dev, torch.float32).contiguous()
        for c0 in range(0, L - 1, 64):
            self._prefill_chunk(x[c0:min(L - 1, c0 + 64)], c0, slot)
        self.x_in[slot].copy_(x[L - 1])
        st = torch.tensor([L - 1, 0, 0, 0, min_len, max_len, seq_id, 0], dtype=torch.int32)
        self.state[:, slot].copy_(st)
        self.sampled[slot].fill_(-1)

    def start(self, lm_inputs: List[torch.Tensor], min_lens: List[int], max_lens: List[int], seed=0, seq_ids=None,
              forced: Optional[torch.Tensor] = None, want_logp=False):
        B = self.B
        assert len(lm_inputs) == B
        self.seed, self.want_logp = int(seed), want_logp
        if forced is not None:
            if self._forced_buf is None:
                self._forced_buf = torch.zeros(B, self.max_out, dtype=torch.int32, device=self.dev)
            self._forced_buf[:, :forced.shape[1]].copy_(forced.to(torch.int32))
            self.forced = self._forced_buf
        else:
            self.forced = None
        st = torch.zeros(8, B, dtype=torch.int32)
        for b in range(B):
            st[ST_MINLEN, b], st[ST_MAXLEN, b] = min_lens[b], max_lens[b]
            st[ST_SEQ, b] = b if seq_ids is None else seq_ids[b]
        self.state.copy_(st)
        self.sampled.fill_(-1)
        for b, x in enumerate(lm_inputs):
            assert x.shape[0] + max_lens[b] <= self.max_pages * self.page, "sequence exceeds the KV cache"
            self.release(b)
            self._set_pages(b, x.shape[0] + min(max_lens[b], self.reserve_ahead))
        if (B >= 4 or self.wplanes or self.h2) and self.pf_layers:
            self._prefill_batch(lm_inputs)
            lm_inputs = []
        for b, x in enumerate(lm_inputs):
            L = x.shape[0]
            x = x.to(self.dev, torch.float32).contiguous()
            for c0 in range(0, L, 64):
                c1 = min(L, c0 + 64)
                hc, hca = self._prefill_chunk(x[c0:c1], c0, b)
            self.h[b].copy_(hc[-1])
            self.h_act[b].copy_(hca[-1])
            self.state[ST_POS, b] = L - 1
        self._tail(B)
        if self._decode is None:
            self._decode = Graphed(self._decode_step, self.use_graphs)
        elif self._graph_key != (self.forced is None, want_logp, self.seed):
            self._decode.release()
            self._decode = Graphed(self._decode_step, self.use_graphs)
        self._graph_key = (self.forced is None, want_logp, self.seed)

    def _prefill_batch(self, lm_inputs):
        B, dt, H, I = self.B, self.dtype, self.H, self.I
        Ls = [int(x.shape[0]) for x in lm_inputs]
        Lm = max(Ls)
        R = B * Lm
        h = torch.zeros(B, Lm, H, device=self.dev)
        for b, x in enumerate(lm_inputs):
            h[b, :Ls[b]].copy_(x)
        h = h.reshape(R, H)
        self._gemm_layers(h, B, Lm, torch.zeros(B, dtype=torch.int32, device=self.dev), self.block_table)
        last = torch.tensor([b * Lm + Ls[b] - 1 for b in range(B)], dtype=torch.long, device=self.dev)
        hl = h.index_select(0, last)
        self.h[:B].copy_(hl)
        self.h_act[:B].copy_(hl)
        self.state[ST_POS].copy_(torch.tensor([L - 1 for L in Ls], dtype=torch.int32))

    def _gemm_layers(self, h, B, Lm, pos, block_table):
        dt, H, I = self.dtype, self.H, self.I
        R = B * Lm
        a = torch.empty(R, H, dtype=self.tdt, device=self.dev)
        qkv = torch.empty(R, (self.Hq + 2 * self.Hkv) * self.D, device=self.dev)
        q = torch.empty(R, self.Hq * self.D, dtype=self.tdt, device=self.dev)
        att = torch.empty(R, self.Hq * self.D, dtype=self.tdt, device=self.dev)
        gu = torch.empty(R, 2 * I, device=self.dev)
        act = torch.empty(R, I, dtype=self.tdt, device=self.dev)
        for l, (w, ws) in enumerate(zip(self.pf_layers, self.layers)):
            ops.rownorm(h, w["g1"], None, self.eps, rows=R, C_=H, rms=True, out_act=a, dtype=dt)
            ops.linear(a, w["wqkv"], H, dtype=dt, bias=ws["bqkv"], out_f32=qkv)
            ops.rope_kv_store(qkv, self.inv_freq, pos, q, self.kc[l], self.vc[l], block_table, B=B, rows=Lm,
                              Hq=self.Hq, Hkv=self.Hkv, page=self.page, dtype=dt)
            ops.paged_attn(q, pos, self.kc[l], self.vc[l], block_table, att, B=B, rows=Lm, Hq=self.Hq,
                           Hkv=self.Hkv, page=self.page, dtype=dt)
            ops.linear(att, w["wo"], self.Hq * self.D, dtype=dt, residual=h, out_f32=h)
            ops.rownorm(h, w["g2"], None, self.eps, rows=R, C_=H, rms=True, out_act=a, dtype=dt)
            ops.linear(a, w["wgu"], H, dtype=dt, out_f32=gu)
            ops.swiglu(gu, act, rows=R, I=I, dtype=dt)
            ops.linear(act, w["wdown"], I, dtype=dt, residual=h, out_f32=h)

    def _prefill_chunk(self, xc, pos0, b):
        rows = xc.shape[0]
        if self.h2 or self.wplanes:
            hc = xc.to(self.dev, torch.float32).clone()
            self._gemm_layers(hc, 1, rows, torch.tensor([pos0], dtype=torch.int32, device=self.dev), self.block_table[b:b + 1].contiguous())
            return hc, hc.to(self.tdt)
        if not self.use_graphs:
            hc = xc.clone()
            hca = hc.to(self.tdt)
            pos = torch.tensor([pos0], dtype=torch.int32, device=self.dev)
            self._layers(hc, hca, 1, rows, pos, self.block_table[b:b + 1])
            return hc, hca
        if not hasattr(self, "_pf"):
            self._pf = dict(h=torch.zeros(64, self.H, device=self.dev), ha=torch.zeros(64, self.H, dtype=self.tdt, device=self.dev),
                            pos=torch.zeros(1, dtype=torch.int32, device=self.dev),
                            bt=torch.zeros(1, self.max_pages, dtype=torch.int32, device=self.dev), graphs={})
        pf = self._pf
        pf["h"][:rows].copy_(xc)
        pf["ha"][:rows].copy_(xc)
        pf["pos"].fill_(pos0)
        pf["bt"].copy_(self.block_table[b:b + 1])
        if rows not in pf["graphs"]:
            pf["graphs"][rows] = Graphed(lambda r=rows: self._layers(pf["h"][:r], pf["ha"][:r], 1, r, pf["pos"], pf["bt"]), True)
        pf["graphs"][rows]()
        return pf["h"][:rows], pf["ha"][:rows]

    def step(self):
        self._decode()

    def close(self):
        if self._decode is not None:
            self._decode.release()
            self._decode = None
        if hasattr(self, "_pf"):
            for g in self._pf["graphs"].values():
                g.release()
            del self._pf

    @torch.no_grad()
    def forward_rows(self, x: torch.Tensor, pos0: int) -> torch.Tensor:
        n = x.shape[0]
        if pos0 + n > self.max_pages * self.page:
            raise RuntimeError("sequence exceeds the KV cache")
        x = x.to(self.dev, torch.float32).contiguous()
        if pos0 == 0:
            self.release(0)
        self._set_pages(0, pos0 + n)
        out = torch.empty(n, self.H, device=self.dev)
        for c0 in range(0, n, 64):
            c1 = min(n, c0 + 64)
            hc, _ = self._prefill_chunk(x[c0:c1], pos0 + c0, 0)
            ops.rownorm(hc, self.norm_w, None, self.eps, rows=c1 - c0, C_=self.H, rms=True, out_f32=out[c0:c1], dtype=F32)
        return out

    def compact_from(self, big: "LlmEngine", idx: List[int]):
        n = len(idx)
        assert n <= self.B and big.kc is self.kc
        ii = torch.tensor(idx, dtype=torch.long, device=self.dev)
        st = torch.zeros(8, self.B, dtype=torch.int32, device=self.dev)
        st[ST_FIN, n:] = 1
        st[:, :n] = big.state[:, ii]
        self.state.copy_(st)
        self.out_tokens[:n].copy_(big.out_tokens[ii])
        self.sampled[:n].copy_(big.sampled[ii])
        self.x_in[:n].copy_(big.x_in[ii])
        self.block_table.fill_(self.trash_page)
        self.block_table[:n].copy_(big.block_table[ii])
        self.seed, self.want_logp = big.seed, False
        self.top_p, self.top_k, self.win_size, self.tau_r = big.top_p, big.top_k, big.win_size, big.tau_r
        self.forced = None
        key = (True, False, self.seed)
        self._fresh_decode_graph(key)

    def _fresh_decode_graph(self, key):
        if self._decode is None or getattr(self, "_graph_key", None) != key:
            if self._decode is not None:
                self._decode.release()
            self._decode = Graphed(self._decode_step, self.use_graphs)
        self._graph_key = key

    def run(self, max_steps: int, poll_every: int = 8) -> List[List[int]]:
        done = 1
        while done < max_steps:
            n = min(poll_every, max_steps - done)
            if self.reserve_ahead < (1 << 30):
                self.ensure_capacity(n + 1)
            for _ in range(n):
                self._decode()
            done += n
            if bool(self.state[ST_FIN].all().item()):
                break
        return self.tokens()

    @torch.no_grad()
    def run_queue(self, requests, seed=0, poll_every: int = 8, ahead: int = 32):
        self.seed, self.want_logp, self.forced = int(seed), False, None
        self._fresh_decode_graph((True, False, self.seed))
        st = torch.zeros(8, self.B, dtype=torch.int32)
        st[ST_FIN] = 1
        self.state.copy_(st)
        for s_ in range(self.B):
            self.release(s_)
        out: List[Optional[List[int]]] = [None] * len(requests)
        owner = [-1] * self.B
        nxt = 0
        while True:
            fin = self.state[ST_FIN].tolist()
            nout = self.state[ST_NOUT].tolist()
            for s_ in range(self.B):
                if owner[s_] >= 0 and fin[s_]:
                    out[owner[s_]] = self.out_tokens[s_, :nout[s_]].tolist()
                    owner[s_] = -1
                    self.release(s_)
                if owner[s_] < 0 and nxt < len(requests):
                    x, mn, mx = requests[nxt]
                    self.admit(s_, x, mn, mx, seq_id=nxt, ahead=ahead + poll_every)
                    owner[s_] = nxt
                    nxt += 1
            active = [s_ for s_ in range(self.B) if owner[s_] >= 0]
            if not active:
                return out
            self.ensure_capacity(ahead + poll_every, active=active)
            for _ in range(poll_every):
                self._decode()

    def open_stream(self, seed=0, seq_id=0, want_logp=False):
        assert self.B == 1, "bistream decode is single-sequence (cli/model.py:105-112)"
        self.release(0)
        self._set_pages(0, self.max_pages * self.page)
        self.seed, self.want_logp, self.forced = int(seed), bool(want_logp), None
        self._st = dict(rows=0, calls=0, hist=0, seq=int(seq_id), last=None)
        self.sampled.fill_(-1)
        self._fresh_decode_graph((True, self.want_logp, self.seed))

    def embed_text(self, tok: torch.Tensor) -> torch.Tensor:
        tok = tok.reshape(-1).to(self.dev, torch.int64)
        x = torch.empty(tok.numel(), self.H, device=self.dev)
        if tok.numel():
            ops.gather_rows(tok, self.embed_tokens, out_f32=x, dtype=F32)
        return x

    def embed_speech(self, tok: torch.Tensor) -> torch.Tensor:
        tok = tok.reshape(-1).to(self.dev, torch.int64)
        x = torch.empty(tok.numel(), self.H, device=self.dev)
        if tok.numel():
            ops.gather_rows(tok, self.speech_emb, out_f32=x, dtype=F32)
        return x

    def _upload_state(self, pos, ignore_eos):
        s = self._st
        st = torch.tensor([pos, s["calls"], s["hist"], 0, (1 << 30) if ignore_eos else 0, 1 << 30, s["seq"], 0],
                          dtype=torch.int32).reshape(8, 1)
        self.state.copy_(st)

    def feed(self, x: Optional[torch.Tensor], ignore_eos: bool) -> int:
        s = self._st
        n = 1 if x is None else x.shape[0]
        if s["rows"] + n > self.max_pages * self.page or s["calls"] >= self.max_out:
            raise RuntimeError("bistream: sequence exceeds the KV cache (no fill token / eos was produced)")
        if x is None:
            self._upload_state(s["rows"], ignore_eos)
            self._decode()
        else:
            x = x.to(self.dev, torch.float32).contiguous()
            for c0 in range(0, n, 64):
                c1 = min(n, c0 + 64)
                hc, hca = self._prefill_chunk(x[c0:c1], s["rows"] + c0, 0)
            self.h[0].copy_(hc[-1])
            self.h_act[0].copy_(hca[-1])
            self._upload_state(s["rows"] + n - 1, ignore_eos)
            self._tail(1)
        tok = int(self.sampled[0, s["calls"]].item())
        if int(self.state[7, 0].item()):
            raise RuntimeError("sampling reaches max_trials 100 and still get eos when ignore_eos is True, check your input!")
        s["rows"] += n
        s["calls"] += 1
        self._last_sampled = tok
        return tok

    def commit(self, token: int):
        s = self._st
        if token != self._last_sampled or token >= self.eos:
            self.out_tokens[0, s["hist"]] = token
            if token < self.eos:
                self.x_in[0].copy_(self.speech_emb[token])
            elif self._last_sampled < self.eos and s["last"] is not None:
                self.x_in[0].copy_(self.speech_emb[s["last"]])
        if token < self.eos:
            s["last"] = token
        s["hist"] += 1

    def tokens(self) -> List[List[int]]:
        n = self.state[ST_NOUT].tolist()
        t = self.out_tokens.cpu()
        return [t[b, :n[b]].tolist() for b in range(self.B)]
```

minimax-speech_amd/mmx/ops.py:

```python
import ctypes as C
import math

import torch

from . import _lib as L
from ._lib import ACT, BF16, F32, check, i64, load, stream, _p


def round_up(x, m):
    return (x + m - 1) // m * m


class Planed(torch.Tensor):
    """A packed weight held as bf16 PLANES hi + [mid +] lo = w of an fp32 checkpoint's values (include/mmx_hip.h MMX_X2W / MMX_X3W).
    The type is the marker: gemm() / skinny2() switch to the weight-plane dtype code when they are handed one; views and row
    slices keep the type (torch's default __torch_function__)."""


def weight_planes(w: torch.Tensor, n: int):
    out, r = [], w.float()
    for _ in range(n):
        t = r.to(torch.bfloat16)
        out.append(t)
        r = r - t.float()
    return out


def resolve_wplanes(wplanes, weights) -> bool:
    if wplanes != "auto":
        return bool(wplanes)
    for w in weights:
        w = w.detach().float()
        if bool(((w - w.to(torch.bfloat16).float()).abs() > 2.0 ** -16 * w.abs()).any()):
            return True
    return False


def pack_linear(w: torch.Tensor, dtype) -> torch.Tensor:
    N, K = w.shape
    Kp = round_up(K, 32)
    planes = L.WPLANES.get(dtype, 1)
    out = torch.zeros(N, planes * Kp, dtype=L.WEIGHT_DT[dtype], device=w.device)
    if planes == 1:
        out[:, :K] = w
        return out
    for i, t in enumerate(weight_planes(w, planes)):
        out[:, i * Kp:i * Kp + K] = t
    return out.as_subclass(Planed)


def conv1d_matrix(w: torch.Tensor) -> torch.Tensor:
    Cout, Cin, k = w.shape
    return w.permute(0, 2, 1).reshape(Cout, k * Cin)


def pack_conv1d(w: torch.Tensor, dtype) -> torch.Tensor:
    return pack_linear(conv1d_matrix(w), dtype)


def pack_convtranspose1d(w: torch.Tensor, stride: int, dtype) -> torch.Tensor:
    Cin, Cout, k = w.shape
    s = stride
    assert k == 2 * s
    wk = w.permute(2, 1, 0)
    tap0 = wk[s:2 * s]
    tap1 = wk[0:s]
    g = torch.cat([tap0, tap1], dim=2)
    return pack_linear(g.reshape(s * Cout, 2 * Cin), dtype)


def fold_weight_norm(g, v):
    n = v.reshape(v.shape[0], -1).norm(dim=1).reshape(-1, *([1] * (v.dim() - 1)))
    return g * (v / n)


def gemm(A, W, M, N, *, dtype, lda=None, cin=None, ntaps=1, dil=1, row_off=0, row_lo=0, row_hi=None, batch=1,
         a_bstride=0, w_bstride=0, bias=None, bias_mod=None, bias_per_row=False, act="none", act2="none", slope=0.1,
         residual=None, ldr=0, r_bstride=0, rowmask=None, rm_bstride=0, alpha=None, alpha_mod=None,
         out_f32=None, ldo_f=0, of_bstride=0, out_act=None, ldo_a=0, oa_bstride=0, out_off=0, out_len=None, row_stride=1,
         tile=0):
    ldw = W.shape[-1] if hasattr(W, "shape") else None
    assert ldw is not None
    if isinstance(W, Planed):
        dtype = {L.X2: L.X2W, L.X3: L.X3W, L.X2W: L.X2W, L.X3W: L.X3W}[dtype]
    elif dtype in L.WPLANES:
        raise L.MmxError("a weight-plane dtype needs a Planed weight (ops.pack_linear with X2W / X3W)")
    p = L.gemm_params(A=A, W=W, bias=bias, residual=residual, rowmask=rowmask, alpha=alpha, out_f32=out_f32,
                      out_act=out_act, lda=lda, ldw=ldw, ldr=ldr, ldo_f=ldo_f, ldo_a=ldo_a,
                      a_bstride=a_bstride, w_bstride=w_bstride, r_bstride=r_bstride, rm_bstride=rm_bstride,
                      of_bstride=of_bstride, oa_bstride=oa_bstride, row_off=row_off, row_lo=row_lo,
                      row_hi=(row_hi if row_hi is not None else (1 << 40)), out_off=out_off,
                      out_len=(out_len if out_len is not None else (1 << 62)), M=M, N=N, batch=batch,
                      ntaps=ntaps, cin=cin, dil=dil, bias_mod=(bias_mod or N), alpha_mod=(alpha_mod or N),
                      bias_per_row=int(bias_per_row), act=ACT[act], act2=ACT[act2], slope=slope, row_stride=row_stride)
    L.gemm_win(p, dtype, tile)


def linear(x, Wp, K, *, dtype, bias=None, act="none", act2="none", residual=None, rowmask=None, out_f32=None,
           out_act=None):
    N = Wp.shape[0]
    M = x.numel() // x.shape[-1]
    gemm(x, Wp, M, N, dtype=dtype, lda=x.shape[-1], cin=K, bias=bias, act=act, act2=act2,
         residual=residual, ldr=N, rowmask=rowmask, out_f32=out_f32, ldo_f=N, out_act=out_act, ldo_a=N)


def conv1d(x, Wp, *, T, Cin, k, dtype, dil=1, pad_left=0, batch=1, bias=None, act="none", slope=0.1, residual=None,
           rowmask=None, alpha=None, out_f32=None, out_act=None, T_out=None, act2="none", stride=1):
    Cout = Wp.shape[0]
    T_out = T if T_out is None else T_out
    gemm(x, Wp, T_out, Cout, dtype=dtype, lda=Cin, cin=Cin, ntaps=k, dil=dil, row_off=-pad_left, row_lo=0, row_hi=T, row_stride=stride,
         batch=batch, a_bstride=T * Cin, bias=bias, act=act, act2=act2, slope=slope,
         residual=residual, ldr=Cout, r_bstride=T_out * Cout, rowmask=rowmask, rm_bstride=T_out,
         alpha=alpha, out_f32=out_f32, ldo_f=Cout, of_bstride=T_out * Cout,
         out_act=out_act, ldo_a=Cout, oa_bstride=T_out * Cout)


def convtranspose1d(x, Wp, *, T, Cin, Cout, stride, dtype, batch=1, bias=None, alpha=None, out_f32=None, out_act=None):
    s = stride
    pad = math.ceil(s / 2)
    gemm(x, Wp, T + 1, s * Cout, dtype=dtype, lda=Cin, cin=Cin, ntaps=2, dil=1, row_off=-1, row_lo=0, row_hi=T,
         batch=batch, a_bstride=T * Cin, bias=bias, bias_mod=Cout, alpha=alpha, alpha_mod=Cout,
         out_f32=out_f32, ldo_f=s * Cout, of_bstride=T * s * Cout, out_act=out_act, ldo_a=s * Cout,
         oa_bstride=T * s * Cout, out_off=-pad * Cout, out_len=T * s * Cout)


def rownorm(x, gamma, beta, eps, *, rows, C_, batch=1, x_bstride=None, rms=False, act="none", rowmask=None,
            addvec=None, av_bstride=None, out_f32=None, out_act=None, dtype=F32, ldx=None, o_bstride=None, rm_bstride=None):
    ldx = C_ if ldx is None else ldx
    xb = rows * ldx if x_bstride is None else x_bstride
    ob = rows * C_ if o_bstride is None else o_bstride
    check(load().mmx_rownorm(_p(x), i64(ldx), i64(xb), rows, C_, batch, _p(gamma), _p(beta), C.c_float(eps), int(rms),
                             ACT[act], _p(rowmask), i64(rows if rm_bstride is None else rm_bstride), _p(addvec),
                             i64(C_ if av_bstride is None else av_bstride), _p(out_f32), i64(C_), i64(ob), _p(out_act), i64(C_),
                             i64(ob), dtype, stream()), "mmx_rownorm")


def groupnorm(x, gamma, beta, out, *, B, T, C_, groups, dtype, eps=1e-5, act="none", rowmask=None):
    check(load().mmx_groupnorm(_p(x), B, T, C_, groups, _p(gamma), _p(beta), C.c_float(eps), ACT[act], _p(rowmask), _p(out),
                               dtype, stream()), "mmx_groupnorm")


def act_rows(x, *, rows, C_, act="none", rowmask=None, out_f32=None, out_act=None, dtype=F32):
    check(load().mmx_act_rows(_p(x), i64(rows), C_, ACT[act], _p(rowmask), _p(out_f32), _p(out_act), dtype, stream()),
          "mmx_act_rows")


def mask_rows(x, rowmask, *, rows, C_, dtype):
    check(load().mmx_mask_rows(_p(x), i64(rows), C_, _p(rowmask), dtype, stream()), "mmx_mask_rows")


def gather_rows(ids, table, *, scale=1.0, rowmask=None, out_f32=None, out_act=None, dtype=F32):
    n, C_ = ids.numel(), table.shape[1]
    check(load().mmx_gather_rows(_p(ids), n, _p(table), C_, C.c_float(scale), _p(rowmask), _p(out_f32), i64(C_),
                                 _p(out_act), i64(C_), dtype, stream()), "mmx_gather_rows")


def copy2d(src, src_dt, ibs, irs, ics, dst, dst_dt, obs, ors, ocs, rows, cols, batch=1, rep=1):
    check(load().mmx_copy2d(_p(src), src_dt, i64(ibs), i64(irs), i64(ics), rep, _p(dst), dst_dt, i64(obs), i64(ors),
                            i64(ocs), rows, cols, batch, stream()), "mmx_copy2d")


def est_pack(x, mu, spks, cond, h, *, B, T, dtype, x_bstride=None, x_mod=None):
    check(load().mmx_est_pack(_p(x), i64(T * 80 if x_bstride is None else x_bstride), (B if x_mod is None else x_mod), _p(mu), _p(spks), _p(cond), B, T, 80, _p(h), i64(h.shape[-1]), dtype, stream()),
          "mmx_est_pack")


def sinusoidal_emb(t, out, *, dim, dtype, scale=1000.0):
    check(load().mmx_sinusoidal_emb(_p(t), t.numel(), dim, C.c_float(scale), _p(out), dtype, stream()),
          "mmx_sinusoidal_emb")


def cfg_euler(x, d_cond, d_uncond, cfg, dt, n):
    check(load().mmx_cfg_euler(_p(x), _p(d_cond), _p(d_uncond), C.c_float(cfg), C.c_float(dt), i64(n), stream()),
          "mmx_cfg_euler")


def conv_cin1(x, w, bias, *, T, C_, k, batch, dtype, slope=0.1, alpha=None, out_f32=None, out_act=None):
    check(load().mmx_conv_cin1(_p(x), i64(T), T, C_, k, _p(w), _p(bias), C.c_float(slope), _p(alpha), _p(out_f32), _p(out_act),
                               batch, dtype, stream()), "mmx_conv_cin1")


def vae_sample(ml, noise, z, m, logs, *, rows, D):
    check(load().mmx_vae_sample(_p(ml), _p(noise), i64(rows), D, _p(z), _p(m), _p(logs), stream()), "mmx_vae_sample")


def prefetch4(tensors, sink, workgroups=128):
    t = list(tensors) + [None] * (4 - len(tensors))
    nb = lambda x: 0 if x is None else (x.numel() * x.element_size()) // 16 * 16
    check(load().mmx_prefetch4(_p(t[0]), i64(nb(t[0])), _p(t[1]), i64(nb(t[1])), _p(t[2]), i64(nb(t[2])), _p(t[3]), i64(nb(t[3])),
                               _p(sink), workgroups, stream()), "mmx_prefetch4")


def resample_linear(x, T2):
    x = x.contiguous()
    T = x.shape[-1]
    out = torch.empty(*x.shape[:-1], T2, dtype=torch.float32, device=x.device)
    check(load().mmx_resample_linear(_p(x), i64(x.numel() // T), T, T2, _p(out), stream()), "mmx_resample_linear")
    return out


def conv_cout1_tanh(act, w, bias, out, *, T, C_, k, batch, dtype, slope=0.1, use_tanh=True):
    check(load().mmx_conv_cout1_tanh(_p(act), i64(T * C_), T, C_, k, _p(w), _p(bias), C.c_float(slope), int(use_tanh),
                                     _p(out), i64(T), batch, dtype, stream()), "mmx_conv_cout1_tanh")


def est_next(wqkv=None, n1g=None, n1b=None, q_out=None, ldq=0, q_bs=0, vt_out=None, ldvt=0, vt_bs=0):
    return L.fill_struct(L.EstNext(), wqkv=wqkv, n1g=n1g, n1b=n1b, q_out=q_out, vt_out=vt_out, q_bs=q_bs, vt_bs=vt_bs,
                         ldq=ldq, ldvt=ldvt)


def est_tail(ao, x, w, *, B, T, dtype, bm, rowmask=None, act_out=None, act_ld=0, nxt=None, eps=1e-5, pf=0, t_begin=0,
             Tcap=None, waves=0, occ2=False, narrow=False):
    Tc = T if Tcap is None else Tcap
    p = L.fill_struct(L.EstTailParams(), ao=ao, x=x, wo=w["wo_p"], w1=w["w1_p"], w2=w["w2_p"], bo=w["bo"], b1=w["b1"],
                      b2=w["b2"], n3g=w["n3g"], n3b=w["n3b"], rowmask=rowmask, act_out=act_out, ao_bs=Tc * 512,
                      x_bs=Tc * 256, rm_bs=Tc, act_bs=Tc * act_ld, ldao=512, act_ld=act_ld, B=B, T=T, t_begin=t_begin, eps=eps)
    if nxt is not None:
        p.next = nxt
    if isinstance(w["wo_p"], Planed):
        dtype = L.X2W
    check(load().mmx_est_tail(C.byref(p), C.c_int(dtype), C.c_int(bm), C.c_int(pf + 16 * waves + (256 if occ2 else 0) + (512 if narrow else 0)), stream()),
          "mmx_est_tail")


def est_resnet(a_in, lda, cin, x, r, tv, tv_bs, *, B, T, dtype, bm, rowmask=None, nxt=None, eps=1e-5, pf=0, t_begin=0,
               Tcap=None, waves=0):
    Tc = T if Tcap is None else Tcap
    p = L.fill_struct(L.EstResnetParams(), a_in=a_in, x=x, w1=r["w1_p"], w2=r["w2_p"], wr=r["wr_p"], b1=r["b1"], g1=r["g1"],
                      be1=r["be1"], b2=r["b2"], g2=r["g2"], be2=r["be2"], br=r["br"], tv=tv, rowmask=rowmask,
                      a_bs=Tc * lda, x_bs=Tc * 256, tv_bs=tv_bs, rm_bs=Tc, lda=lda, cin=cin, B=B, T=T, t_begin=t_begin, eps=eps)
    if nxt is not None:
        p.next = nxt
    if isinstance(r["w1_p"], Planed):
        dtype = L.X2W
    check(load().mmx_est_resnet(C.byref(p), C.c_int(dtype), C.c_int(bm), C.c_int(pf + 16 * waves), stream()), "mmx_est_resnet")


def pack_dac_ru(w7: torch.Tensor, w1: torch.Tensor, dtype):
    C_ = w7.shape[0]
    CP = (C_ + 31) // 32 * 32
    wd = torch.float32 if dtype in L.WPLANES else L.WEIGHT_DT[dtype]
    a = torch.zeros(C_, 7, CP, dtype=torch.float32, device=w7.device)
    a[:, :, :C_] = w7.permute(0, 2, 1)
    b = torch.zeros(C_, CP, dtype=torch.float32, device=w7.device)
    b[:, :C_] = w1[:, :, 0]
    return (pack_skinny(a.reshape(C_, 7 * CP).to(wd).contiguous(), dtype=dtype), pack_skinny(b.to(wd).contiguous(), dtype=dtype))


def dac_ru(x, x_out, ru, *, B, T, C_, dil, dtype, act_out=None, alpha_next=None, lens=None, bm=0, slope=0.1, x_bs=None):
    p = L.fill_struct(L.DacRuParams(), x=x, x_out=x_out, act_out=act_out, w7=ru["w7_p"], w1=ru["w1_p"], b7=ru["b7"], b1=ru["b1"],
                      a0=ru["a0"], a2=ru["a2"], alpha_next=alpha_next, lens=lens, x_bs=(T * C_ if x_bs is None else x_bs),
                      B=B, T=T, C=C_, dil=dil, slope=slope)
    if isinstance(ru["w7_p"], Planed):
        dtype = L.X2W
    check(load().mmx_dac_ru(C.byref(p), C.c_int(dtype), C.c_int(bm), stream()), "mmx_dac_ru")


def attn_dense(q, k, v, out, *, B, H, Tq, Tk, ldq, ldk, ldv, ldo, q_bs, k_bs, v_bs, o_bs, scale, dtype,
               keymask=None, chunk=0, pos=None, ldp=0, pos_u=None, pos_v=None, head_stride=0, q_begin=0, km_bs=None):
    check(load().mmx_attn_dense(_p(q), i64(ldq), i64(q_bs), _p(k), i64(ldk), i64(k_bs), _p(v), i64(ldv), i64(v_bs),
                                _p(out), i64(ldo), i64(o_bs), B, H, 64, Tq, Tk, C.c_float(scale), _p(keymask),
                                i64(Tk if km_bs is None else km_bs), chunk, _p(pos), i64(ldp), _p(pos_u), _p(pos_v), head_stride,
                                q_begin, dtype, stream()),
          "mmx_attn_dense")


def attn_relpos_bf16(q, k, vt, pos, pos_u, pos_v, out, *, B, H, T, ldq, ldk, ldvt, ldp, ldo, q_bs, k_bs, vt_bs, o_bs, scale, chunk=0,
                     klen=None):
    if klen is not None:
        assert klen.dtype == torch.int32 and klen.numel() >= B
    check(load().mmx_attn_relpos_bf16(_p(q), i64(ldq), i64(q_bs), _p(k), i64(ldk), i64(k_bs), _p(vt), i64(ldvt), i64(vt_bs),
                                      _p(pos), i64(ldp), _p(pos_u), _p(pos_v), _p(out), i64(ldo), i64(o_bs), B, H, T,
                                      C.c_float(scale), chunk, _p(klen), stream()), "mmx_attn_relpos_bf16")


def attn_relpos_x(q, k, v, pos, pos_u, pos_v, out, *, B, H, T, ldq, ldk, ldv, ldp, ldo, q_bs, k_bs, v_bs, o_bs, scale, chunk=0, klen=None):
    if klen is not None:
        assert klen.dtype == torch.int32 and klen.numel() >= B
    check(load().mmx_attn_relpos_x(_p(q), i64(ldq), i64(q_bs), _p(k), i64(ldk), i64(k_bs), _p(v), i64(ldv), i64(v_bs), _p(pos), i64(ldp),
                                   _p(pos_u), _p(pos_v), _p(out), i64(ldo), i64(o_bs), B, H, T, C.c_float(scale), chunk, _p(klen), stream()),
          "mmx_attn_relpos_x")


def attn_flash_bf16(q, k, vt, out, *, B, H, T, ldq, ldk, ldvt, ldo, q_bs, k_bs, vt_bs, o_bs, scale, keymask=None,
                    chunk=0, q_begin=0, km_bs=None, fp8=False, klen=None):
    if klen is not None:
        assert klen.dtype == torch.int32 and klen.numel() >= B
    if fp8:
        check(load().mmx_attn_flash_fp8(_p(q), i64(ldq), i64(q_bs), _p(k), i64(ldk), i64(k_bs), _p(vt), i64(ldvt),
                                        i64(vt_bs), _p(out), i64(ldo), i64(o_bs), B, H, T, C.c_float(scale),
                                        _p(keymask), i64(T if km_bs is None else km_bs), chunk, q_begin, _p(klen), stream()), "mmx_attn_flash_fp8")
        return
    check(load().mmx_attn_flash_bf16(_p(q), i64(ldq), i64(q_bs), _p(k), i64(ldk), i64(k_bs), _p(vt), i64(ldvt),
                                     i64(vt_bs), _p(out), i64(ldo), i64(o_bs), B, H, T, C.c_float(scale),
                                     _p(keymask), i64(T if km_bs is None else km_bs), chunk, q_begin, _p(klen), stream()), "mmx_attn_flash_bf16")


def attn_flash_x(q, k, v, out, *, B, H, T, ldq, ldk, ldv, ldo, q_bs, k_bs, v_bs, o_bs, scale, keymask=None, chunk=0, q_begin=0,
                 km_bs=None, klen=None):
    if klen is not None:
        assert klen.dtype == torch.int32 and klen.numel() >= B
    check(load().mmx_attn_flash_x(_p(q), i64(ldq), i64(q_bs), _p(k), i64(ldk), i64(k_bs), _p(v), i64(ldv), i64(v_bs),
                                  _p(out), i64(ldo), i64(o_bs), B, H, T, C.c_float(scale), _p(keymask),
                                  i64(T if km_bs is None else km_bs), chunk, q_begin, _p(klen), stream()), "mmx_attn_flash_x")


def attn_flash_xs(qk, vt, out, *, B, H, T, ldqk, ldvt, ldo, qk_bs, vt_bs, o_bs, scale, keymask=None, chunk=0, q_begin=0, km_bs=None,
                  klen=None, form=0):
    if klen is not None:
        assert klen.dtype == torch.int32 and klen.numel() >= B
    check(load().mmx_attn_flash_xs(_p(qk), i64(ldqk), i64(qk_bs), _p(vt), i64(ldvt), i64(vt_bs), _p(out), i64(ldo), i64(o_bs), B, H, T,
                                   C.c_float(scale), _p(keymask), i64(T if km_bs is None else km_bs), chunk, q_begin, _p(klen), int(form),
                                   stream()), "mmx_attn_flash_xs")


def pack_skinny(w, *, dtype, kscale=None, interleave_half=0):
    N, K = w.shape
    if dtype in L.WPLANES:
        assert w.dtype == torch.float32 and kscale is None
        base = {L.X2W: L.X2, L.X3W: L.X3}[dtype]
        return torch.cat([pack_skinny(t.contiguous(), dtype=base, interleave_half=interleave_half)
                          for t in weight_planes(w, L.WPLANES[dtype])]).as_subclass(Planed)
    assert w.dtype == L.WEIGHT_DT[dtype]
    KB = 32 if L.WEIGHT_DT[dtype] == torch.bfloat16 else 16
    tiles = (N + 15) // 16
    wp = torch.empty(tiles * (K // KB) * 64 * (KB // 4), dtype=L.WEIGHT_DT[dtype], device=w.device)
    check(load().mmx_pack_skinny(_p(w), i64(w.stride(0)), N, K, _p(kscale), interleave_half, _p(wp), dtype, stream()),
          "mmx_pack_skinny")
    return wp


X_PACKED, OUT_PACKED = 1, 2


def packed_rows(B):
    return (B + 15) // 16 * 16


def pack_act(x, dtype):
    E = 8 if dtype == BF16 else 4
    B, K = x.shape
    R = packed_rows(B)
    xp = torch.zeros(R, K, dtype=x.dtype, device=x.device)
    xp[:B] = x
    return xp.reshape(R // 16, 16, K // (4 * E), 4, E).permute(0, 2, 3, 1, 4).contiguous().reshape(-1)


def unpack_act(xp, B, K, dtype):
    E = 8 if dtype == BF16 else 4
    R = packed_rows(B)
    return xp.reshape(R // 16, K // (4 * E), 4, 16, E).permute(0, 3, 1, 2, 4).reshape(R, K)[:B]


def skinny_gemm(x, wp, *, B, K, N, dtype, bias=None, rs=False, eps=1e-6, epi=0, out_f32=None, out_act=None,
                ldx=None, ldo_f=None, ldo_a=None, x_packed=False, out_packed=False, kgamma=None):
    xdt = L.dt_of(x)
    flags = (X_PACKED if x_packed else 0) | (OUT_PACKED if out_packed else 0)
    check(load().mmx_skinny_gemm(_p(x), xdt, i64(ldx if ldx is not None else K), B, K, N, _p(wp), _p(bias), int(rs),
                                 C.c_float(eps), epi, _p(out_f32), i64(ldo_f if ldo_f is not None else N),
                                 _p(out_act), i64(ldo_a if ldo_a is not None else N), dtype, flags, _p(kgamma), stream()),
          "mmx_skinny_gemm")


SSQ_SLOTS = 64


def plane_elems(B, K):
    return packed_rows(B) * K


def split_planes(x, f16=False):
    B, K = x.shape
    out, r = [], x.float()
    for _ in range(2 if f16 else 3):
        t = r.to(torch.float16 if f16 else torch.bfloat16)
        out.append(pack_act(t.view(torch.bfloat16) if f16 else t, BF16))
        r = r - t.float()
    return torch.stack(out)


def merge_planes(xs, B, K, f16=False):
    if f16:
        return sum(unpack_act(xs[s], B, K, BF16).contiguous().view(torch.float16).float() for s in range(2))
    return sum(unpack_act(xs[s], B, K, BF16).float() for s in range(3))


H2_WSCALE = 256.0


def pack_skinny_h2(w, *, planes=1, interleave_half=0):
    ws = w.float() * H2_WSCALE
    assert float(ws.abs().max()) < 65504.0, "weight out of the fp16 range of MMX_H2"
    out, r = [], ws
    for _ in range(planes):
        t = r.to(torch.float16)
        out.append(pack_skinny(t.view(torch.bfloat16).contiguous(), dtype=L.X3, interleave_half=interleave_half))
        r = r - t.float()
    return out[0] if planes == 1 else torch.cat(out).as_subclass(Planed)


def decode_prep(x, xs, ssq, *, B, K, gamma=None, h=None, dtype=L.X3):
    check(load().mmx_decode_prep(_p(x), i64(x.shape[-1]), B, K, _p(gamma), _p(h), i64(h.shape[-1] if h is not None else 0), _p(xs),
                                 _p(ssq), dtype, stream()), "mmx_decode_prep")


def skinny2(xs, wp, *, B, K, N, dtype, bias=None, ssq_in=None, eps=1e-6, epi=0, out=None, ldo=None, xs_out=None, gamma_next=None,
            ssq_out=None, tiles_per_wg=1, ksplit=1, part=None, tickets=None):
    if isinstance(wp, Planed):
        dtype = L.H2W if dtype in (L.H2, L.H2W) else L.X3W
    check(load().mmx_skinny2(_p(xs), B, K, N, _p(wp), _p(bias), _p(ssq_in), C.c_float(eps), epi, _p(out),
                             i64(ldo if ldo is not None else N), _p(xs_out), _p(gamma_next), _p(ssq_out), tiles_per_wg, ksplit,
                             _p(part), i64(part.numel() if part is not None else 0), _p(tickets), dtype, stream()), "mmx_skinny2")


def rope_kv_store(qkv, inv_freq, pos, q_out, kc, vc, block_table, *, B, rows, Hq, Hkv, page, dtype):
    ld = (Hq + 2 * Hkv) * 64
    check(load().mmx_rope_kv_store(_p(qkv), i64(ld), i64(rows * ld), B, rows, Hq, Hkv, 64, _p(inv_freq), _p(pos),
                                   _p(q_out), i64(Hq * 64), i64(rows * Hq * 64), _p(kc), _p(vc), _p(block_table),
                                   block_table.shape[1], page, dtype, stream()), "mmx_rope_kv_store")


def paged_attn(q, pos, kc, vc, block_table, out, *, B, rows, Hq, Hkv, page, dtype):
    check(load().mmx_paged_attn(_p(q), i64(Hq * 64), i64(rows * Hq * 64), B, rows, Hq, Hkv, 64, C.c_float(0.125),
                                _p(pos), _p(kc), _p(vc), _p(block_table), block_table.shape[1], page, _p(out),
                                i64(Hq * 64), i64(rows * Hq * 64), dtype, stream()), "mmx_paged_attn")


def decode_attn(qkv, inv_freq, pos, kc, vc, block_table, out, *, B, Hq, Hkv, page, dtype, rope_tab=None, out_packed=False,
                per_head=False, out_split=False, one_head=False):
    check(load().mmx_decode_attn(_p(qkv), i64((Hq + 2 * Hkv) * 64), B, Hq, Hkv, 64, _p(inv_freq), _p(rope_tab), _p(pos), _p(kc),
                                 _p(vc), _p(block_table), block_table.shape[1], page, C.c_float(0.125), _p(out),
                                 i64(Hq * 64), dtype, int(bool(out_packed)) | (2 if per_head else 0) | (8 if out_split == "f16" else (4 if out_split else 0)) | (16 if one_head else 0), stream()), "mmx_decode_attn")


def swiglu(gu, out, *, rows, I, dtype):
    check(load().mmx_swiglu(_p(gu), i64(2 * I), rows, I, _p(out), i64(I), dtype, stream()), "mmx_swiglu")


def sample_step(logits, state, out_tokens, speech_emb, next_x, *, V, B, eos_id, seed, top_k=25, top_p=0.8,
                win_size=10, tau_r=0.1, sampled=None, forced=None, logp_out=None):
    check(load().mmx_sample_step(_p(logits), i64(logits.shape[-1]), V, B, eos_id, top_k, C.c_float(top_p), win_size,
                                 C.c_float(tau_r), C.c_uint64(seed), _p(state), _p(out_tokens), out_tokens.shape[1],
                                 _p(sampled), _p(forced), _p(speech_emb), speech_emb.shape[1], _p(next_x),
                                 i64(next_x.shape[-1]), _p(logp_out), stream()), "mmx_sample_step")
```

Baseline: 546.3.

## Fuse weight prefetch into decode kernels via extra prefetch workgroups instead of side stream

Replaces the side-stream prefetch4 launches, each guarded by per-layer events, with extra workgroups appended to the skinny GEMM and decode-attention grids. These workgroups stream slices of upcoming weights into cache, following a fixed plan that spreads each layer's weights across the preceding kernels. The aim is to hide weight load latency for the next kernels without the cost of extra streams and event syncs. In exchange, the prefetch blocks compete with the compute blocks for CUs and bandwidth, and the grid and partial-buffer indexing had to be reworked to use the compute tile count.

```diff
diff --git a/include/mmx_hip.h b/include/mmx_hip.h
--- a/include/mmx_hip.h
+++ b/include/mmx_hip.h
@@ -136,6 +136,15 @@
                 int epi, float* out, int64_t ldo, void* xs_out, const float* gamma_next, float* ssq_out,
                 int tiles_per_wg, int ksplit, float* part, int64_t part_floats, int32_t* tickets, int dtype,
                 hipStream_t stream);
+typedef struct MmxPrefetchDesc {
+    const void* p0; int64_t n0;
+    const void* p1; int64_t n1;
+    int32_t workgroups;
+} MmxPrefetchDesc;
+int mmx_skinny2_pf(const void* xs, int B, int K, int N, const void* wp, const float* bias, const float* ssq_in, float eps,
+                   int epi, float* out, int64_t ldo, void* xs_out, const float* gamma_next, float* ssq_out,
+                   int tiles_per_wg, int ksplit, float* part, int64_t part_floats, int32_t* tickets, int dtype,
+                   const MmxPrefetchDesc* pf, hipStream_t stream);
 
 int mmx_rope_kv_store(const float* qkv, int64_t ldqkv, int64_t qkv_bs, int B, int rows, int Hq, int Hkv, int D,
                       const float* inv_freq, const int32_t* pos, void* q_out, int64_t ldq, int64_t q_bs,
@@ -147,6 +156,9 @@
 int mmx_decode_attn(const float* qkv, int64_t ldqkv, int B, int Hq, int Hkv, int D, const float* inv_freq,
                     const float* rope_tab, const int32_t* pos, void* kc, void* vc, const int32_t* block_table, int max_pages, int page,
                     float scale, void* out, int64_t ldo, int dtype, int out_packed, hipStream_t stream);
+int mmx_decode_attn_pf(const float* qkv, int64_t ldqkv, int B, int Hq, int Hkv, int D, const float* inv_freq,
+                       const float* rope_tab, const int32_t* pos, void* kc, void* vc, const int32_t* block_table, int max_pages, int page,
+                       float scale, void* out, int64_t ldo, int dtype, int out_packed, const MmxPrefetchDesc* pf, hipStream_t stream);
 int mmx_swiglu(const float* gu, int64_t ldgu, int rows, int I, void* out, int64_t ldo, int dtype, hipStream_t stream);
 
 int mmx_sample_step(const float* logits, int64_t ldl, int V, int B, int eos_id, int top_k, float top_p,
diff --git a/minimax-speech_amd/csrc/common.h b/minimax-speech_amd/csrc/common.h
--- a/minimax-speech_amd/csrc/common.h
+++ b/minimax-speech_amd/csrc/common.h
@@ -184,3 +184,42 @@
     float s = PRECISE ? sin_cw(alpha * x) : __sinf(alpha * x);
     return x + (1.0f / (alpha + 1e-9f)) * (s * s);
 }
+
+struct PfRole {
+    const uint4* p[2];
+    unsigned n16[2];
+    int first, nwg;
+};
+template <int NT>
+__device__ __forceinline__ void prefetch_role(const PfRole& r, int wg) {
+    constexpr int U = 8;
+    if (wg >= r.nwg) return;
+    unsigned acc = 0;
+#pragma unroll
+    for (int k = 0; k < 2; ++k) {
+        const unsigned n = r.n16[k], per = (n + r.nwg - 1) / (unsigned)r.nwg;
+        const unsigned lo = min(n, wg * per), hi = min(n, lo + per);
+        for (unsigned i = lo + threadIdx.x; i < hi; i += NT * U) {
+            uint4 v[U];
+#pragma unroll
+            for (int u = 0; u < U; ++u) {
+                const unsigned j = i + u * NT;
+                v[u] = j < hi ? r.p[k][j] : make_uint4(0, 0, 0, 0);
+            }
+#pragma unroll
+            for (int u = 0; u < U; ++u) acc ^= v[u].x ^ v[u].y ^ v[u].z ^ v[u].w;
+        }
+    }
+    asm volatile("" ::"v"(acc));
+}
+inline bool pf_role_make(PfRole& r, const void* p0, int64_t n0, const void* p1, int64_t n1, int wgs, int first) {
+    if (wgs < 0 || wgs > 1024 || n0 < 0 || n1 < 0 || n0 > (int64_t)1 << 31 || n1 > (int64_t)1 << 31) return false;
+    if (((uintptr_t)p0 % 16) != 0 || ((uintptr_t)p1 % 16) != 0) return false;
+    r.p[0] = (const uint4*)p0;
+    r.p[1] = (const uint4*)p1;
+    r.n16[0] = p0 ? (unsigned)(n0 >> 4) : 0u;
+    r.n16[1] = p1 ? (unsigned)(n1 >> 4) : 0u;
+    r.first = first;
+    r.nwg = (r.n16[0] | r.n16[1]) ? wgs : 0;
+    return true;
+}
diff --git a/minimax-speech_amd/csrc/decode.hip b/minimax-speech_amd/csrc/decode.hip
--- a/minimax-speech_amd/csrc/decode.hip
+++ b/minimax-speech_amd/csrc/decode.hip
@@ -53,13 +53,16 @@
     float eps;
     unsigned wplane;
     float wscale;
+    PfRole pf;
 };
 
 __device__ unsigned long long* g_skinny_stamps = nullptr;
-#define STAMP(i) do { if constexpr (LAB) { if (stamps && lane == 0) stamps[((blockIdx.y * gridDim.x + blockIdx.x) * 8 + wave) * 8 + (i)] = __builtin_amdgcn_s_memtime(); } } while (0)
+#define STAMP(i) do { if constexpr (LAB) { if (stamps && lane == 0) stamps[((blockIdx.y * ntx + blockIdx.x) * 8 + wave) * 8 + (i)] = __builtin_amdgcn_s_memtime(); } } while (0)
 
 template <int MT, int TW, int KPW, int EPI, int NS, int NWP = 1, bool F16 = false>
 __global__ __launch_bounds__(512) void skinny3_kernel(Skinny3Args a) {
+    const int ntx = a.pf.first;
+    if ((int)blockIdx.x >= ntx) { prefetch_role<512>(a.pf, ((int)blockIdx.x - ntx) * (int)gridDim.y + (int)blockIdx.y); return; }
     unsigned long long* stamps = nullptr;
     unsigned long long t_entry = 0;
     if constexpr (LAB) { t_entry = __builtin_amdgcn_s_memtime(); stamps = g_skinny_stamps; }
@@ -80,7 +83,7 @@
     const int ntiles = a.ntiles;
 
     STAMP(0);
-    if constexpr (LAB) { if (stamps && lane == 0) stamps[((blockIdx.y * gridDim.x + blockIdx.x) * 8 + wave) * 8 + 7] = t_entry; }
+    if constexpr (LAB) { if (stamps && lane == 0) stamps[((blockIdx.y * ntx + blockIdx.x) * 8 + wave) * 8 + 7] = t_entry; }
     const auto w_rsrc = __builtin_amdgcn_make_buffer_rsrc(const_cast<bf16_t*>(a.wp), 0, 0x7fffffff, 0x00020000);
     const auto x_rsrc = __builtin_amdgcn_make_buffer_rsrc(const_cast<bf16_t*>(a.xs), 0, 0x7fffffff, 0x00020000);
     const unsigned voff = lane * 16;
@@ -183,7 +186,7 @@
 #pragma unroll
             for (int k = 0; k < UPW; ++k) {
                 const int u = wave + 8 * k;
-                if (u < UNITS) st_sc1(a.part + ((j * gridDim.x + blockIdx.x) * UNITS + u) * 64 + lane, sum[k][0]);
+                if (u < UNITS) st_sc1(a.part + ((j * ntx + blockIdx.x) * UNITS + u) * 64 + lane, sum[k][0]);
             }
             asm volatile("s_waitcnt vmcnt(0)" ::: "memory");
             __syncthreads();
@@ -202,7 +205,7 @@
 #pragma unroll
                 for (int j2 = 0; j2 < JMAX; ++j2) {
                     const int u = min(wave + 8 * k, UNITS - 1), jc = min(j2, J - 1);
-                    const float v = ld_sc1(a.part + ((jc * gridDim.x + blockIdx.x) * UNITS + u) * 64 + lane);
+                    const float v = ld_sc1(a.part + ((jc * ntx + blockIdx.x) * UNITS + u) * 64 + lane);
                     pv[k][j2] = j2 < J ? v : 0.f;
                 }
 #pragma unroll
@@ -247,7 +250,7 @@
     constexpr int NB = EPI == 1 ? 2 : 1;
     const size_t lds = (size_t)8 * (TW * NB * MT * 4) * 64 * sizeof(float) + 32 * sizeof(float) + 16;
     MMX_LDS_OPT_IN((skinny3_kernel<MT, TW, KPW, EPI, NS, NWP, F16>), lds);
-    dim3 grid((a.ntiles + TW - 1) / TW, J);
+    dim3 grid(a.pf.first + (a.pf.nwg + J - 1) / J, J);
     hipLaunchKernelGGL((skinny3_kernel<MT, TW, KPW, EPI, NS, NWP, F16>), grid, dim3(512), lds, s, a);
     MMX_LAUNCH_CHECK();
     return MMX_OK;
@@ -284,10 +287,10 @@
     return MMX_OK;
 }
 
-extern "C" int mmx_skinny2(const void* xs, int B, int K, int N, const void* wp, const float* bias, const float* ssq_in, float eps,
-                           int epi, float* out, int64_t ldo, void* xs_out, const float* gamma_next, float* ssq_out,
-                           int tiles_per_wg, int ksplit, float* part, int64_t part_floats, int32_t* tickets, int dtype,
-                           hipStream_t stream) {
+extern "C" int mmx_skinny2_pf(const void* xs, int B, int K, int N, const void* wp, const float* bias, const float* ssq_in, float eps,
+                              int epi, float* out, int64_t ldo, void* xs_out, const float* gamma_next, float* ssq_out,
+                              int tiles_per_wg, int ksplit, float* part, int64_t part_floats, int32_t* tickets, int dtype,
+                              const MmxPrefetchDesc* pf, hipStream_t stream) {
     MMX_CHECK_ARG(xs && wp && B > 0 && B <= 32 && K > 0 && K % 32 == 0 && N > 0 &&
                   (dtype == MMX_X3 || dtype == MMX_X3W || dtype == MMX_BF16 || dtype == MMX_H2 || dtype == MMX_H2W));
     MMX_CHECK_ARG(dtype != MMX_X3W || tiles_per_wg == 1);
@@ -302,8 +305,12 @@
     const double plane_bytes = (double)ntiles * (epi == 1 ? 2 : 1) * nkb * 1024.0;
     MMX_CHECK_ARG(plane_bytes * (dtype == MMX_X3W ? 3 : (dtype == MMX_H2W ? 2 : 1)) < 2147483000.0);
     const bool f16 = dtype == MMX_H2 || dtype == MMX_H2W;
+    MMX_CHECK_ARG(tiles_per_wg == 1 || tiles_per_wg == 2);
+    PfRole role;
+    MMX_CHECK_ARG(pf_role_make(role, pf ? pf->p0 : nullptr, pf ? pf->n0 : 0, pf ? pf->p1 : nullptr, pf ? pf->n1 : 0, pf ? pf->workgroups : 0,
+                               (ntiles + tiles_per_wg - 1) / tiles_per_wg));
     Skinny3Args a{(const bf16_t*)xs, (const bf16_t*)wp, bias, ssq_in, out, (bf16_t*)xs_out, gamma_next, ssq_out, part, tickets,
-                  ldo, B, K, N, ntiles, (nkb + ksplit - 1) / ksplit, eps, (unsigned)plane_bytes, f16 ? 1.0f / H2_WSCALE : 1.0f};
+                  ldo, B, K, N, ntiles, (nkb + ksplit - 1) / ksplit, eps, (unsigned)plane_bytes, f16 ? 1.0f / H2_WSCALE : 1.0f, role};
 #define GO(MT, TW, KPW, EPI) do { if (dtype == MMX_X3) return launch<MT, TW, KPW, EPI, 3>(a, ksplit, stream); \
                                   if (dtype == MMX_H2) return launch<MT, TW, KPW, EPI, 2, 1, true>(a, ksplit, stream); \
                                   if (dtype == MMX_H2W) return launch<MT, TW, KPW, EPI, 2, 2, true>(a, ksplit, stream); \
@@ -320,6 +327,14 @@
     return MMX_EARG;
 }
 
+extern "C" int mmx_skinny2(const void* xs, int B, int K, int N, const void* wp, const float* bias, const float* ssq_in, float eps,
+                           int epi, float* out, int64_t ldo, void* xs_out, const float* gamma_next, float* ssq_out,
+                           int tiles_per_wg, int ksplit, float* part, int64_t part_floats, int32_t* tickets, int dtype,
+                           hipStream_t stream) {
+    return mmx_skinny2_pf(xs, B, K, N, wp, bias, ssq_in, eps, epi, out, ldo, xs_out, gamma_next, ssq_out, tiles_per_wg, ksplit, part,
+                          part_floats, tickets, dtype, nullptr, stream);
+}
+
 #if MMX_LAB
 extern "C" int mmx_lab_skinny_stamps(void* buf) {
     unsigned long long* p = reinterpret_cast<unsigned long long*>(buf);
diff --git a/minimax-speech_amd/csrc/llm.hip b/minimax-speech_amd/csrc/llm.hip
--- a/minimax-speech_amd/csrc/llm.hip
+++ b/minimax-speech_amd/csrc/llm.hip
@@ -522,7 +522,8 @@
     const float* __restrict__ qkv, long ldqkv, int Hq, int Hkv, const float* __restrict__ inv_freq,
     const float* __restrict__ rope_tab, const int32_t* __restrict__ pos, T* __restrict__ kc, T* __restrict__ vc,
     const int32_t* __restrict__ block_table, int max_pages, int page, float scale, T* __restrict__ out, long ldo,
-    int nseq) {
+    int nseq, PfRole pf) {
+    if ((int)blockIdx.x >= pf.first) { prefetch_role<256>(pf, (int)blockIdx.x - pf.first); return; }
     constexpr int D = 64, HALF = 32, NG = 32;
     extern __shared__ __attribute__((aligned(16))) char smem[];
     float* qs = reinterpret_cast<float*>(smem);
@@ -883,9 +884,10 @@
         out[OPK ? act_packed_index<bf16_t>(b, col, Hq * D) : (long)b * ldo + col] = f2bf(o / L);
     }
 }
-extern "C" int mmx_decode_attn(const float* qkv, int64_t ldqkv, int B, int Hq, int Hkv, int D, const float* inv_freq,
-                               const float* rope_tab, const int32_t* pos, void* kc, void* vc, const int32_t* block_table, int max_pages,
-                               int page, float scale, void* out, int64_t ldo, int dtype, int out_packed, hipStream_t stream) {
+extern "C" int mmx_decode_attn_pf(const float* qkv, int64_t ldqkv, int B, int Hq, int Hkv, int D, const float* inv_freq,
+                                  const float* rope_tab, const int32_t* pos, void* kc, void* vc, const int32_t* block_table, int max_pages,
+                                  int page, float scale, void* out, int64_t ldo, int dtype, int out_packed, const MmxPrefetchDesc* pf,
+                                  hipStream_t stream) {
     dtype = MMX_ACT_DTYPE(dtype);
     MMX_CHECK_ARG(qkv && (inv_freq || rope_tab) && pos && kc && vc && block_table && out && B > 0 && D == 64 && Hq % Hkv == 0 && page > 0);
     MMX_CHECK_ARG(out_packed >= 0 && out_packed <= 31);
@@ -900,10 +902,14 @@
     const int hp = one_head ? 1 : 2, nsub = (Hq / Hkv + hp - 1) / hp;
     size_t lds = ((size_t)hp * 64 + 2 * 64 + 2 * hp * 32 + (size_t)hp * 32 * 64 + (size_t)max_pages) * 4;
     MMX_CHECK_ARG(lds <= 64 * 1024);
-    dim3 grid(8 * ((Hkv * B + 7) / 8) * nsub);
-#define DA(T, OM) do { if (one_head) hipLaunchKernelGGL((decode_attn_kernel<T, OM, 1>), grid, dim3(256), lds, stream, qkv, ldqkv, Hq, Hkv, inv_freq, rope_tab, pos, (T*)kc, (T*)vc, block_table, max_pages, page, scale, (T*)out, ldo, B); \
-                       else hipLaunchKernelGGL((decode_attn_kernel<T, OM, 2>), grid, dim3(256), lds, stream, qkv, ldqkv, Hq, Hkv, inv_freq, rope_tab, pos, (T*)kc, (T*)vc, block_table, max_pages, page, scale, (T*)out, ldo, B); } while (0)
+    const int ncompute = 8 * ((Hkv * B + 7) / 8) * nsub;
+    PfRole role;
+    MMX_CHECK_ARG(pf_role_make(role, pf ? pf->p0 : nullptr, pf ? pf->n0 : 0, pf ? pf->p1 : nullptr, pf ? pf->n1 : 0, pf ? pf->workgroups : 0, ncompute));
+    dim3 grid(ncompute + role.nwg);
+#define DA(T, OM) do { if (one_head) hipLaunchKernelGGL((decode_attn_kernel<T, OM, 1>), grid, dim3(256), lds, stream, qkv, ldqkv, Hq, Hkv, inv_freq, rope_tab, pos, (T*)kc, (T*)vc, block_table, max_pages, page, scale, (T*)out, ldo, B, role); \
+                       else hipLaunchKernelGGL((decode_attn_kernel<T, OM, 2>), grid, dim3(256), lds, stream, qkv, ldqkv, Hq, Hkv, inv_freq, rope_tab, pos, (T*)kc, (T*)vc, block_table, max_pages, page, scale, (T*)out, ldo, B, role); } while (0)
     if (dtype == MMX_BF16 && page == 16 && Hq == 7 * Hkv && gqa_shared) {
+        MMX_CHECK_ARG(role.nwg == 0);
         const size_t lds2 = (2 * 16 * 64 + 2 * 64) * 2 + (4 * 8 * 16 * 8 + 3 * 32 + 32 * 7 * 64 + (size_t)max_pages) * 4;
         MMX_CHECK_ARG(lds2 <= 160 * 1024);
         if (out_packed) MMX_LDS_OPT_IN((decode_attn_gqa_kernel<true, 7>), lds2);
@@ -916,3 +922,9 @@
     MMX_LAUNCH_CHECK();
     return MMX_OK;
 }
+extern "C" int mmx_decode_attn(const float* qkv, int64_t ldqkv, int B, int Hq, int Hkv, int D, const float* inv_freq,
+                               const float* rope_tab, const int32_t* pos, void* kc, void* vc, const int32_t* block_table, int max_pages,
+                               int page, float scale, void* out, int64_t ldo, int dtype, int out_packed, hipStream_t stream) {
+    return mmx_decode_attn_pf(qkv, ldqkv, B, Hq, Hkv, D, inv_freq, rope_tab, pos, kc, vc, block_table, max_pages, page, scale, out, ldo,
+                              dtype, out_packed, nullptr, stream);
+}
diff --git a/minimax-speech_amd/mmx/_lib.py b/minimax-speech_amd/mmx/_lib.py
--- a/minimax-speech_amd/mmx/_lib.py
+++ b/minimax-speech_amd/mmx/_lib.py
@@ -24,7 +24,7 @@
 SYMBOLS = [
     "mmx_abi_version", "mmx_gemm_win", "mmx_gemm_win_tile", "mmx_rownorm", "mmx_groupnorm", "mmx_act_rows", "mmx_gather_rows", "mmx_copy2d", "mmx_est_pack",
     "mmx_sinusoidal_emb", "mmx_cfg_euler", "mmx_attn_dense", "mmx_attn_flash_bf16", "mmx_attn_flash_fp8", "mmx_attn_relpos_bf16", "mmx_attn_relpos_x", "mmx_attn_flash_x", "mmx_attn_flash_xs", "mmx_conv_cout1_tanh", "mmx_conv_cin1", "mmx_vae_sample", "mmx_resample_linear", "mmx_prefetch4", "mmx_mask_rows",
-    "mmx_est_tail", "mmx_est_resnet", "mmx_dac_ru", "mmx_pack_skinny", "mmx_skinny_gemm", "mmx_skinny2", "mmx_decode_prep", "mmx_rope_kv_store", "mmx_paged_attn", "mmx_decode_attn", "mmx_swiglu", "mmx_sample_step",
+    "mmx_est_tail", "mmx_est_resnet", "mmx_dac_ru", "mmx_pack_skinny", "mmx_skinny_gemm", "mmx_skinny2", "mmx_skinny2_pf", "mmx_decode_prep", "mmx_rope_kv_store", "mmx_paged_attn", "mmx_decode_attn", "mmx_decode_attn_pf", "mmx_swiglu", "mmx_sample_step",
 ]
 
 
@@ -64,6 +64,10 @@
 class DacRuParams(C.Structure):
     _fields_ = [(k, C.c_void_p) for k in ("x", "x_out", "act_out", "w7", "w1", "b7", "b1", "a0", "a2", "alpha_next", "lens")] + \
                [("x_bs", C.c_int64)] + [(k, C.c_int32) for k in ("B", "T", "C", "dil")] + [("slope", C.c_float)]
+
+
+class PrefetchDesc(C.Structure):
+    _fields_ = [("p0", C.c_void_p), ("n0", C.c_int64), ("p1", C.c_void_p), ("n1", C.c_int64), ("workgroups", C.c_int32)]
 
 
 def fill_struct(st, **kw):
diff --git a/minimax-speech_amd/mmx/llm.py b/minimax-speech_amd/mmx/llm.py
--- a/minimax-speech_amd/mmx/llm.py
+++ b/minimax-speech_amd/mmx/llm.py
@@ -178,6 +178,32 @@
                             x_packed=pk, out_packed=pk)
 
     v2_cfg = dict(qkv=(1, 1), o=(1, 1), gu=(2, 1), down=(2, 8), head=(2, 1))
+    pf_plan = (("qkv", "wo", 0.0, 1.0), ("qkv", "wgu", 0.0, 0.5),
+               ("attn", "wgu", 0.5, 1.0),
+               ("o", "wdown", 0.0, 0.7),
+               ("gu", "wdown", 0.7, 1.0),
+               ("down", "next", 0.0, 1.0))
+    pf_max_wgs = 512
+
+    def _pf_descs(self):
+        kb = int(self.prefetch)
+        key = (kb, self.pf_plan, self.pf_max_wgs)
+        if getattr(self, "_pf_key", None) != key:
+            out = []
+            for l, w in enumerate(self.layers if kb else []):
+                nxt = self.layers[l + 1]["wqkv"] if l + 1 < len(self.layers) else self.wdec
+                rows = {}
+                for carrier, name, f0, f1 in self.pf_plan:
+                    t = nxt if name == "next" else w[name]
+                    if t is None:
+                        continue
+                    nb = t.numel() * t.element_size()
+                    b0, b1 = int(nb * f0) // 1024 * 1024, (nb if f1 >= 1.0 else int(nb * f1) // 1024 * 1024)
+                    if b1 > b0:
+                        rows.setdefault(carrier, []).append((t, b0, b1 - b0))
+                out.append({c: ops.prefetch_desc(r, min(self.pf_max_wgs, max(1, -(-sum(x[2] for x in r) // (kb * 1024))))) for c, r in rows.items()})
+            self._pf_list, self._pf_key = out, key
+        return self._pf_list
 
     def _planes(self):
         if not hasattr(self, "_v2"):
@@ -196,36 +222,21 @@
         NQ = (self.Hq + 2 * self.Hkv) * self.D
         qkv = S["qkv"][:B]
         ops.decode_prep(x_in, S["xs_a"], S["ssq_a"], B=B, K=H, gamma=self.layers[0]["g1"], h=h, dtype=dt)
-        pf = int(self.prefetch)
-        if pf:
-            if not hasattr(self, "_pf_side"):
-                self._pf_side = torch.cuda.Stream(device=self.dev)
-                self._pf_sink = torch.zeros(4, dtype=torch.int32, device=self.dev)
-            cur, side = torch.cuda.current_stream(), self._pf_side
+        pfs = self._pf_descs()
         for l, w in enumerate(self.layers):
-            if pf:
-                nxt = self.layers[l + 1] if l + 1 < len(self.layers) else None
-                ev = torch.cuda.Event()
-                ev.record(cur)
-                side.wait_event(ev)
-                with torch.cuda.stream(side):
-                    ops.prefetch4([nxt["wqkv"], nxt["wo"], nxt["wgu"], nxt["wdown"]] if nxt is not None else [self.wdec], self._pf_sink, pf)
+            pf = pfs[l] if pfs else {}
             g_next = self.layers[l + 1]["g1"] if l + 1 < len(self.layers) else self.norm_w
             ops.skinny2(S["xs_a"], w["wqkv"], B=B, K=H, N=NQ, dtype=dt, bias=w["bqkv"], ssq_in=S["ssq_a"], eps=self.eps, epi=0, out=qkv,
-                        tiles_per_wg=c["qkv"][0])
+                        tiles_per_wg=c["qkv"][0], prefetch=pf.get("qkv"))
             ops.decode_attn(qkv, self.inv_freq, pos, self.kc[l], self.vc[l], block_table, S["xs_att"], B=B, Hq=self.Hq,
                             Hkv=self.Hkv, page=self.page, dtype=self.dtype, rope_tab=self.rope_tab, per_head=(self.split or B < self.gqa_min_batch),
-                            out_split=("f16" if self.h2 else self.split), out_packed=not self.split)
+                            out_split=("f16" if self.h2 else self.split), out_packed=not self.split, prefetch=pf.get("attn"))
             ops.skinny2(S["xs_att"], w["wo"], B=B, K=self.Hq * self.D, N=H, dtype=dt, epi=2, out=h, xs_out=S["xs_b"],
-                        gamma_next=w["g2"], ssq_out=S["ssq_b"], tiles_per_wg=c["o"][0])
+                        gamma_next=w["g2"], ssq_out=S["ssq_b"], tiles_per_wg=c["o"][0], prefetch=pf.get("o"))
             ops.skinny2(S["xs_b"], w["wgu"], B=B, K=H, N=I, dtype=dt, ssq_in=S["ssq_b"], eps=self.eps, epi=1, xs_out=S["xs_act"],
-                        tiles_per_wg=c["gu"][0])
+                        tiles_per_wg=c["gu"][0], prefetch=pf.get("gu"))
             ops.skinny2(S["xs_act"], w["wdown"], B=B, K=I, N=H, dtype=dt, epi=2, out=h, xs_out=S["xs_a"], gamma_next=g_next,
-                        ssq_out=S["ssq_a"], tiles_per_wg=c["down"][0], ksplit=c["down"][1], part=S["part"], tickets=S["tickets"])
-        if pf:
-            ev = torch.cuda.Event()
-            ev.record(side)
-            cur.wait_event(ev)
+                        ssq_out=S["ssq_a"], tiles_per_wg=c["down"][0], ksplit=c["down"][1], part=S["part"], tickets=S["tickets"], prefetch=pf.get("down"))
 
     def _layers_split(self, h, B, rows, pos, block_table):
         dt, H, I = self.dtype, self.H, self.I
diff --git a/minimax-speech_amd/mmx/ops.py b/minimax-speech_amd/mmx/ops.py
--- a/minimax-speech_amd/mmx/ops.py
+++ b/minimax-speech_amd/mmx/ops.py
@@ -404,13 +404,37 @@
                                  _p(ssq), dtype, stream()), "mmx_decode_prep")
 
 
+def prefetch_desc(ranges, workgroups):
+    assert len(ranges) <= 2
+    d = L.PrefetchDesc(None, 0, None, 0, int(workgroups))
+    for i, r in enumerate(ranges):
+        if r is None:
+            continue
+        if isinstance(r, tuple) and len(r) == 3:
+            t, off, n = r
+            assert t.is_cuda and t.is_contiguous() and 0 <= off and off + n <= t.numel() * t.element_size()
+            p, n = t.data_ptr() + off, n
+        elif isinstance(r, tuple):
+            p, n = r
+        else:
+            assert r.is_cuda and r.is_contiguous()
+            p, n = r.data_ptr(), r.numel() * r.element_size()
+        setattr(d, f"p{i}", p or None)
+        setattr(d, f"n{i}", int(n))
+    return d
+
+
 def skinny2(xs, wp, *, B, K, N, dtype, bias=None, ssq_in=None, eps=1e-6, epi=0, out=None, ldo=None, xs_out=None, gamma_next=None,
-            ssq_out=None, tiles_per_wg=1, ksplit=1, part=None, tickets=None):
+            ssq_out=None, tiles_per_wg=1, ksplit=1, part=None, tickets=None, prefetch=None):
     if isinstance(wp, Planed):
         dtype = L.H2W if dtype in (L.H2, L.H2W) else L.X3W
-    check(load().mmx_skinny2(_p(xs), B, K, N, _p(wp), _p(bias), _p(ssq_in), C.c_float(eps), epi, _p(out),
-                             i64(ldo if ldo is not None else N), _p(xs_out), _p(gamma_next), _p(ssq_out), tiles_per_wg, ksplit,
-                             _p(part), i64(part.numel() if part is not None else 0), _p(tickets), dtype, stream()), "mmx_skinny2")
+    args = (_p(xs), B, K, N, _p(wp), _p(bias), _p(ssq_in), C.c_float(eps), epi, _p(out),
+            i64(ldo if ldo is not None else N), _p(xs_out), _p(gamma_next), _p(ssq_out), tiles_per_wg, ksplit,
+            _p(part), i64(part.numel() if part is not None else 0), _p(tickets), dtype)
+    if prefetch is None:
+        check(load().mmx_skinny2(*args, stream()), "mmx_skinny2")
+    else:
+        check(load().mmx_skinny2_pf(*args, C.byref(prefetch), stream()), "mmx_skinny2_pf")
 
 
 def rope_kv_store(qkv, inv_freq, pos, q_out, kc, vc, block_table, *, B, rows, Hq, Hkv, page, dtype):
@@ -427,10 +451,14 @@
 
 
 def decode_attn(qkv, inv_freq, pos, kc, vc, block_table, out, *, B, Hq, Hkv, page, dtype, rope_tab=None, out_packed=False,
-                per_head=False, out_split=False, one_head=False):
-    check(load().mmx_decode_attn(_p(qkv), i64((Hq + 2 * Hkv) * 64), B, Hq, Hkv, 64, _p(inv_freq), _p(rope_tab), _p(pos), _p(kc),
-                                 _p(vc), _p(block_table), block_table.shape[1], page, C.c_float(0.125), _p(out),
-                                 i64(Hq * 64), dtype, int(bool(out_packed)) | (2 if per_head else 0) | (8 if out_split == "f16" else (4 if out_split else 0)) | (16 if one_head else 0), stream()), "mmx_decode_attn")
+                per_head=False, out_split=False, one_head=False, prefetch=None):
+    args = (_p(qkv), i64((Hq + 2 * Hkv) * 64), B, Hq, Hkv, 64, _p(inv_freq), _p(rope_tab), _p(pos), _p(kc),
+            _p(vc), _p(block_table), block_table.shape[1], page, C.c_float(0.125), _p(out),
+            i64(Hq * 64), dtype, int(bool(out_packed)) | (2 if per_head else 0) | (8 if out_split == "f16" else (4 if out_split else 0)) | (16 if one_head else 0))
+    if prefetch is None:
+        check(load().mmx_decode_attn(*args, stream()), "mmx_decode_attn")
+    else:
+        check(load().mmx_decode_attn_pf(*args, C.byref(prefetch), stream()), "mmx_decode_attn_pf")
 
 
 def swiglu(gu, out, *, rows, I, dtype):
```

After: 536.7. 1.8% lower.
